# TomClabault/RayTracerCPP

Hardware: AMD Instinct MI355X
Metric: Mrays/sec (primary+shadow) at 1920x1080, 1M-tri scene; max |dpixel| (higher is better)
Workload: dtype f32; 1 GPU; C4 sphere1m: 1,000,000 tris, 1920x1080, ssaa_factor 2 (3840x2160 rays), primary + shadow, octree 12/40; rays_per_frame=10029157, primary_rays=8294400, reflection_rays=0, band_rows=8, parallelism=image strips x1, frames_in_flight=3, world_size=1, bands=interleaved b % N

## Files before the change

### __graft_entry__.py

```python
import os
import subprocess
import sys

ROOT = os.path.dirname(os.path.abspath(__file__))


def _make(args, cwd):
    jobs = str(min(8, os.cpu_count() or 1))
    subprocess.run(["make", "-j" + jobs] + args, cwd=cwd, check=True)


def build() -> None:
    _make([], os.path.join(ROOT, "raytracercpp_amd", "csrc"))
    _make([], os.path.join(ROOT, "oracle"))
    if os.path.isdir("/root/reference/tp2"):
        _make(["ref", "ref_v3"], os.path.join(ROOT, "oracle"))
    sys.path.insert(0, ROOT)
    import raytracercpp_amd
    from raytracercpp_amd import _lib
    _lib.lib()
    sys.path.insert(0, os.path.join(ROOT, "tests"))
    from test_c_api import build_c_program
    build_c_program()
    from scene_bound_tool import build_program
    build_program()
    from tile_mask_tool import build_program as build_tile_mask_program
    build_tile_mask_program()
    if os.path.isdir("/root/reference/tp2"):
        from test_reference_adapter import build_adapter_program
        build_adapter_program()


def smoke() -> None:
    sys.path.insert(0, ROOT)
    import numpy as np
    from raytracercpp_amd import scenes
    from raytracercpp_amd.renderer import Renderer
    from oracle.bindings import Oracle

    sc, st = scenes.bumpy70k(width=160, height=90)
    r = Renderer(0)
    r.load_scene(sc, st)
    r.request_aux(hit=True)
    ref = Oracle(sc, st).render_rows()
    for frame in ("octree", "wide BVH"):
        r.ray_trace()
        r.post_process()
        img = r.get_image().ravel()
        gpu = r.get_internal(argb=False, hit=True)
        assert np.array_equal(gpu["hit_id"], ref.hit_id), f"hit-ID mismatch vs oracle ({frame} frame)"
        assert np.array_equal(img, ref.argb), f"ARGB mismatch vs oracle ({frame} frame)"
        r.finish_accel()
    print("smoke OK:", r.stats())
```

### include/rt_mi355x.h

```cpp
#ifndef RT_MI355X_H
#define RT_MI355X_H

#include <stdint.h>

#ifdef __cplusplus
extern "C" {
#endif

#define RT_OK 0
#define RT_EINVAL (-1)
#define RT_EHIP (-2)
#define RT_ENOMEM (-3)
#define RT_ESTATE (-4)
#define RT_EUNSUPPORTED (-5)
#define RT_EIO (-6)

#define RT_SHADING_RT 0
#define RT_SHADING_ABS_NORMALS 1
#define RT_SHADING_PASTEL_NORMALS 2
#define RT_SHADING_BARYCENTRIC 3
#define RT_SHADING_VISUALIZE_AO 4

#define RT_TEX_AO 0
#define RT_TEX_DIFFUSE 1
// ... 114 lines not shown
int rt_get_camera_matrices(rt_renderer *r, float pos[3], float proj_inv[16], float cam_to_world[16]);

int rt_set_camera_projection(rt_renderer *r, const float proj[16], const float world_to_cam[16]);

int rt_set_camera_lens(rt_renderer *r, float fov, float aspect);

int rt_set_object_transform(rt_renderer *r, const float m[16]);
int rt_reset_previous_transform(rt_renderer *r);
int rt_get_triangles(rt_renderer *r, float *tri9, int64_t *n);

int rt_set_texture(rt_renderer *r, int32_t slot, int32_t w, int32_t h, const float *rgba);

int rt_set_skybox(rt_renderer *r, const int32_t w[6], const int32_t h[6], const float *const faces[6]);

int rt_reconstruct_bvh_new(rt_renderer *r);
int rt_destroy_bvh(rt_renderer *r);

int rt_ray_trace(rt_renderer *r);

int rt_raster_trace(rt_renderer *r);

int rt_get_ssao_buffers(rt_renderer *r, float *z, float *n4, int32_t *ao);

int rt_post_process(rt_renderer *r);

int rt_get_image(rt_renderer *r, uint32_t *argb, int32_t *w, int32_t *h);

int rt_lock_image(rt_renderer *r);
int rt_unlock_image(rt_renderer *r);

int rt_render(rt_renderer *r, float *ms);

int rt_request_aux(rt_renderer *r, int32_t want_rgba, int32_t want_hit, int32_t want_shadow);
int rt_get_internal(rt_renderer *r, uint32_t *argb, float *rgba, int32_t *hit_id, float *hit_t, uint8_t *shadow);

int rt_get_stats(rt_renderer *r, rt_stats *out);

int rt_local_rows(rt_renderer *r, int32_t band_rows, int32_t rank, int32_t nranks, int32_t *rows_out);
int rt_render_bands_device(rt_renderer *r, int32_t band_rows, int32_t rank, int32_t nranks, uint32_t *d_out,
                           void *hip_stream);
int rt_render_band_list_device(rt_renderer *r, int32_t band_rows, const int32_t *bands, int32_t nbands,
                               uint32_t *d_out, void *hip_stream);
int rt_band_costs(rt_renderer *r, void *hip_stream, double *costs, int32_t nbands);

int rt_trace_rays(rt_renderer *r, const float *orig, const float *dir, int64_t n, int32_t *tri_id, float *t,
                  float *u, float *v, uint8_t *ret);

int rt_trace_ray(rt_renderer *r, const float *orig, const float *dir, int64_t n, int32_t current_recursion_depth,
                 float *rgba, int32_t *hit_src, float *t, uint8_t *intersection_found, uint8_t *shadowed);

int rt_kernel_times(rt_renderer *r, float *ms, int32_t n);
int rt_band_counters(rt_renderer *r, int64_t *shadow_rays, int64_t *reflection_rays);
int rt_tile_mask(rt_renderer *r, int32_t src, uint32_t *words, int64_t cap, int32_t info[5]);

void rt_make_transform(int32_t kind, float x, float y, float z, float out[16]);
void rt_compose(const float a[16], const float b[16], float out[16]);
void rt_inverse(const float m[16], float out[16]);
void rt_perspective(float fov, float aspect, float znear, float zfar, float out[16]);
void rt_transform_points(const float m[16], const float *pts, int64_t n, float *out);

typedef struct rt_obj rt_obj;
rt_obj *rt_obj_open(const char *path, const float xform[16], int32_t mat_offset);
int rt_obj_counts(const rt_obj *o, int64_t *ntri, int32_t *nmat, int32_t *has_uv);
int rt_obj_fetch(const rt_obj *o, float *tri9, int32_t *mat, float *uv6, float *mats16);
void rt_obj_close(rt_obj *o);


#ifdef __cplusplus
}
#endif
#endif
```

### include/rt_mi355x_diag.h

```cpp
#ifndef RT_MI355X_DIAG_H
#define RT_MI355X_DIAG_H

#include "rt_mi355x.h"

#ifdef __cplusplus
extern "C" {
#endif

int rt_debug_read(rt_renderer *r, uint64_t *out, int64_t n);
int rt_tile_costs(rt_renderer *r, uint32_t *out, int64_t n, int32_t *tiles_x, int32_t *tiles_y);

int rt_wide_query(rt_renderer *r, const float *orig, const float *dir, int64_t n, int32_t kind, float *o_out,
                  float *d_out, int32_t *status, int32_t *tri_id, float *t, float *u, float *v, uint8_t *shadowed);
int rt_risk_words(rt_renderer *r, int32_t src, uint64_t *out, int64_t cap, int64_t *count, int64_t *violations);

int rt_octree_digest(const float *tri9, int64_t n, int32_t max_depth, int32_t leaf_max_obj_count, int32_t builder,
                     uint64_t *digest, int64_t stats[7], float *ms);

int rt_wbvh_query(const float *tri9, int64_t n, int32_t max_depth, int32_t leaf_max_obj_count, const float *orig,
                  const float *dir, int64_t nrays, int32_t *status, int32_t *id, float *t, float *u, float *v,
                  int64_t stats[8], float *ms);
int rt_wbvh_query_ex(const float *tri9, int64_t n, int32_t max_depth, int32_t leaf_max_obj_count, const float *orig,
                     const float *dir, int64_t nrays, const float *cam, const float *light, int32_t shadow_rays,
                     float *o_out, float *d_out, int32_t *status, int32_t *id, float *t, float *u, float *v,
                     int64_t stats[8], float *ms, int32_t *ray_nodes, int32_t ocone_dim, int64_t oc_stats[5]);

int rt_ocone_check(const float *tri9, int64_t n, int32_t max_depth, int32_t leaf_max_obj_count, int32_t ocone_dim,
                   const float *orig, const float *dir, int64_t nrays, int32_t *skip, int64_t out[6],
                   const uint32_t *cells, const int32_t *dims, const float *lo_ih, uint32_t *cells_out);
int rt_ocone_read(rt_renderer *r, uint32_t *out, int64_t n, int32_t dims[3], float lo_ih[4]);
int rt_risk_cap_check(const float *tri9, int64_t n, int32_t max_depth, int32_t leaf_max_obj_count, const float *cam,
                      const float *dir, int64_t nrays, float cap_override, int32_t *skip, int64_t out[4]);

#ifdef __cplusplus
}
#endif
#endif
```

### raytracercpp_amd/_lib.py

```python
from __future__ import annotations

import ctypes as C
import os

import numpy as np

HERE = os.path.dirname(os.path.abspath(__file__))
LIB_PATH = os.path.join(HERE, "librt_mi355x.so")
if os.environ.get("RT_LIB_PATH"):
    LIB_PATH = os.environ["RT_LIB_PATH"]

RT_OK = 0
ERRORS = {-1: "RT_EINVAL", -2: "RT_EHIP", -3: "RT_ENOMEM", -4: "RT_ESTATE", -5: "RT_EUNSUPPORTED", -6: "RT_EIO"}

_f32p = C.POINTER(C.c_float)
_i32p = C.POINTER(C.c_int32)
_u32p = C.POINTER(C.c_uint32)
_u8p = C.POINTER(C.c_uint8)
_i64p = C.POINTER(C.c_int64)


class RtSettings(C.Structure):
    _fields_ = [
        ("image_width", C.c_int32), ("image_height", C.c_int32),
        ("enable_ssaa", C.c_int32), ("ssaa_factor", C.c_int32),
        ("enable_clipping", C.c_int32), ("hybrid_rasterization_tracing", C.c_int32),
        ("shading_method", C.c_int32), ("compute_shadows", C.c_int32), ("max_recursion_depth", C.c_int32),
        ("enable_bvh", C.c_int32), ("bvh_max_depth", C.c_int32), ("bvh_leaf_object_count", C.c_int32),
        ("enable_ssao", C.c_int32), ("ssao_sample_count", C.c_int32),
        ("ssao_radius", C.c_float), ("ssao_amount", C.c_float),
        ("enable_ambient", C.c_int32), ("enable_diffuse", C.c_int32), ("enable_specular", C.c_int32),
        ("enable_emissive", C.c_int32), ("rough_reflections_sample_count", C.c_int32),
        ("enable_ao_mapping", C.c_int32), ("enable_diffuse_mapping", C.c_int32),
        ("enable_normal_mapping", C.c_int32), ("enable_displacement_mapping", C.c_int32),
        ("displacement_mapping_strength", C.c_float), ("parallax_mapping_steps", C.c_int32),
        ("enable_roughness_mapping", C.c_int32), ("enable_skysphere", C.c_int32), ("enable_skybox", C.c_int32),
        ("rng_seed", C.c_uint32),
    ]


class RtStats(C.Structure):
    _fields_ = [
        ("primary_rays", C.c_int64), ("shadow_rays", C.c_int64), ("reflection_rays", C.c_int64),
        ("kernel_ms", C.c_float), ("post_ms", C.c_float), ("build_ms", C.c_float),
        ("octree_inner", C.c_int64), ("octree_leaves", C.c_int64), ("octree_empty_leaves", C.c_int64),
        ("octree_max_leaf", C.c_int64), ("octree_max_depth", C.c_int64),
        ("gpu_nodes", C.c_int64), ("gpu_tris", C.c_int64),
        ("render_width", C.c_int32), ("render_height", C.c_int32), ("seg_scale", C.c_float),
        ("work", C.c_int64 * 4), ("work_wide", C.c_int64 * 4), ("uncertified", C.c_int64 * 6),
        ("wave_steps", C.c_int64 * 6), ("build_split_ms", C.c_float * 4), ("host_builds", C.c_int64),
        ("wide_tree", C.c_int32),
    ]

    def as_dict(self):
        def conv(n, t):
            v = getattr(self, n)
            if t is C.c_float:
                return float(v)
            if isinstance(v, C.Array):
                return [float(x) if n == "build_split_ms" else int(x) for x in v]
            return int(v)
        return {n: conv(n, t) for n, t in self._fields_}


_H = C.c_void_p
SIGNATURES = {
    "rt_default_settings": (None, [C.POINTER(RtSettings)]),
    "rt_create": (_H, [C.c_int]),
    "rt_destroy": (None, [_H]),
    "rt_last_error": (C.c_char_p, []),
    "rt_get_settings": (C.c_int, [_H, C.POINTER(RtSettings)]),
    "rt_set_settings": (C.c_int, [_H, C.POINTER(RtSettings)]),
    "rt_change_render_size": (C.c_int, [_H, C.c_int32, C.c_int32]),
    "rt_set_exact": (C.c_int, [_H, C.c_int]),
    "rt_finish_accel": (C.c_int, [_H]),
    "rt_set_devices": (C.c_int, [_H, _i32p, C.c_int32]),
    "rt_set_triangles": (C.c_int, [_H, _f32p, _i32p, _f32p, C.c_int64]),
    "rt_add_sphere": (C.c_int, [_H, C.c_float, C.c_float, C.c_float, C.c_float, C.c_int32]),
    "rt_add_plane": (C.c_int, [_H] + [C.c_float] * 6 + [C.c_int32]),
    "rt_clear_geometry": (C.c_int, [_H]),
    "rt_set_materials": (C.c_int, [_H, _f32p, C.c_int32]),
    "rt_get_material_count": (C.c_int, [_H, _i32p]),
    "rt_change_camera_fov": (C.c_int, [_H, C.c_float]),
    "rt_change_camera_aspect_ratio": (C.c_int, [_H, C.c_float]),
    "rt_set_light_position": (C.c_int, [_H, C.c_float, C.c_float, C.c_float]),
    "rt_set_camera_transform": (C.c_int, [_H, _f32p]),
    "rt_apply_transformation_to_camera": (C.c_int, [_H, _f32p]),
    "rt_set_camera_matrices": (C.c_int, [_H, _f32p, _f32p, _f32p]),
    "rt_set_camera_projection": (C.c_int, [_H, _f32p, _f32p]),
    "rt_set_camera_lens": (C.c_int, [_H, C.c_float, C.c_float]),
    "rt_get_ssao_buffers": (C.c_int, [_H, _f32p, _f32p, _i32p]),
    "rt_get_camera_matrices": (C.c_int, [_H, _f32p, _f32p, _f32p]),
    "rt_set_object_transform": (C.c_int, [_H, _f32p]),
    "rt_reset_previous_transform": (C.c_int, [_H]),
    "rt_get_triangles": (C.c_int, [_H, _f32p, _i64p]),
    "rt_get_device_transforms": (C.c_int, [_H, _i64p]),
    "rt_transform_points_device": (C.c_int, [C.c_int32, _f32p, _f32p, C.c_int64, _f32p, _i32p, _f32p]),
    "rt_set_triangles_device": (C.c_int, [_H, C.c_void_p, C.c_int64, C.c_void_p, _i32p, _f32p, C.c_int64, C.c_void_p]),
    "rt_update_vertices_device": (C.c_int, [_H, C.c_void_p, C.c_int64, C.c_void_p, C.c_void_p]),
    "rt_get_device_ingests": (C.c_int, [_H, _i64p]),
    "rt_gather_triangles_device": (C.c_int, [C.c_int32, _f32p, C.c_int64, _i32p, C.c_int64, _f32p, _i32p, _f32p]),
    "rt_set_accel_deferred": (C.c_int, [_H, C.c_int]),
    "rt_get_accel_builds": (C.c_int, [_H, _i64p]),
    "rt_set_texture": (C.c_int, [_H, C.c_int32, C.c_int32, C.c_int32, _f32p]),
    "rt_set_skybox": (C.c_int, [_H, _i32p, _i32p, C.POINTER(_f32p)]),
    "rt_reconstruct_bvh_new": (C.c_int, [_H]),
    "rt_destroy_bvh": (C.c_int, [_H]),
    "rt_ray_trace": (C.c_int, [_H]),
    "rt_raster_trace": (C.c_int, [_H]),
    "rt_post_process": (C.c_int, [_H]),
    "rt_get_image": (C.c_int, [_H, _u32p, _i32p, _i32p]),
    "rt_render": (C.c_int, [_H, _f32p]),
    "rt_lock_image": (C.c_int, [_H]),
    "rt_unlock_image": (C.c_int, [_H]),
    "rt_request_aux": (C.c_int, [_H, C.c_int32, C.c_int32, C.c_int32]),
    "rt_get_internal": (C.c_int, [_H, _u32p, _f32p, _i32p, _f32p, _u8p]),
    "rt_get_stats": (C.c_int, [_H, C.POINTER(RtStats)]),
    "rt_local_rows": (C.c_int, [_H, C.c_int32, C.c_int32, C.c_int32, _i32p]),
    "rt_render_bands_device": (C.c_int, [_H, C.c_int32, C.c_int32, C.c_int32, C.c_void_p, C.c_void_p]),
    "rt_render_band_list_device": (C.c_int, [_H, C.c_int32, _i32p, C.c_int32, C.c_void_p, C.c_void_p]),
    "rt_band_costs": (C.c_int, [_H, C.c_void_p, C.POINTER(C.c_double), C.c_int32]),
    "rt_trace_rays": (C.c_int, [_H, _f32p, _f32p, C.c_int64, _i32p, _f32p, _f32p, _f32p, _u8p]),
    "rt_trace_ray": (C.c_int, [_H, _f32p, _f32p, C.c_int64, C.c_int32, _f32p, _i32p, _f32p, _u8p, _u8p]),
    "rt_wide_query": (C.c_int, [_H, _f32p, _f32p, C.c_int64, C.c_int32, _f32p, _f32p, _i32p, _i32p, _f32p, _f32p, _f32p,
                                _u8p]),
    "rt_risk_words": (C.c_int, [_H, C.c_int32, C.POINTER(C.c_uint64), C.c_int64, _i64p, _i64p]),
    "rt_kernel_times": (C.c_int, [_H, _f32p, C.c_int32]),
    "rt_band_counters": (C.c_int, [_H, _i64p, _i64p]),
    "rt_tile_mask": (C.c_int, [_H, C.c_int32, _u32p, C.c_int64, _i32p]),
    "rt_make_transform": (None, [C.c_int32, C.c_float, C.c_float, C.c_float, _f32p]),
    "rt_compose": (None, [_f32p, _f32p, _f32p]),
    "rt_inverse": (None, [_f32p, _f32p]),
    "rt_perspective": (None, [C.c_float, C.c_float, C.c_float, C.c_float, _f32p]),
    "rt_transform_points": (None, [_f32p, _f32p, C.c_int64, _f32p]),
    "rt_obj_open": (_H, [C.c_char_p, _f32p, C.c_int32]),
    "rt_obj_counts": (C.c_int, [_H, _i64p, _i32p, _i32p]),
    "rt_obj_fetch": (C.c_int, [_H, _f32p, _i32p, _f32p, _f32p]),
    "rt_obj_close": (None, [_H]),
    "rt_octree_digest": (C.c_int, [_f32p, C.c_int64, C.c_int32, C.c_int32, C.c_int32, C.POINTER(C.c_uint64), _i64p,
                                   _f32p]),
    "rt_octree_build_device": (C.c_int, [C.c_int32, _f32p, C.c_int64, C.c_int32, C.c_int32, C.POINTER(C.c_uint64),
                                         _i64p, _f32p]),
    "rt_set_device_build": (C.c_int, [_H, C.c_int]),
    "rt_get_device_builds": (C.c_int, [_H, _i64p]),
    "rt_get_device_wide_builds": (C.c_int, [_H, _i64p]),
    "rt_wbvh_quick_digest": (C.c_int, [_f32p, C.c_int64, C.c_int32, C.c_int32, C.POINTER(C.c_uint64), _i64p, _f32p]),
    "rt_wbvh_quick_build_device": (C.c_int, [C.c_int32, _f32p, C.c_int64, C.c_int32, C.c_int32, C.POINTER(C.c_uint64),
                                             _i64p, _i64p, _f32p]),
    "rt_debug_read": (C.c_int, [_H, C.POINTER(C.c_uint64), C.c_int64]),
    "rt_tile_costs": (C.c_int, [_H, C.POINTER(C.c_uint32), C.c_int64, _i32p, _i32p]),
    "rt_wbvh_query": (C.c_int, [_f32p, C.c_int64, C.c_int32, C.c_int32, _f32p, _f32p, C.c_int64, _i32p, _i32p, _f32p,
                                _f32p, _f32p, _i64p, _f32p]),
    "rt_wbvh_query_ex": (C.c_int, [_f32p, C.c_int64, C.c_int32, C.c_int32, _f32p, _f32p, C.c_int64, _f32p, _f32p,
                                   C.c_int32, _f32p, _f32p, _i32p, _i32p, _f32p, _f32p, _f32p, _i64p, _f32p, _i32p,
                                   C.c_int32, _i64p]),
    "rt_ocone_check": (C.c_int, [_f32p, C.c_int64, C.c_int32, C.c_int32, C.c_int32, _f32p, _f32p, C.c_int64, _i32p,
                                 _i64p, C.POINTER(C.c_uint32), _i32p, _f32p, C.POINTER(C.c_uint32)]),
    "rt_ocone_read": (C.c_int, [_H, C.POINTER(C.c_uint32), C.c_int64, _i32p, _f32p]),
    "rt_risk_cap_check": (C.c_int, [_f32p, C.c_int64, C.c_int32, C.c_int32, _f32p, _f32p, C.c_int64, C.c_float, _i32p,
                                    _i64p]),
}

GEOMETRY_INPUT = ("rt_set_triangles_device", "rt_update_vertices_device", "rt_get_device_ingests",
                  "rt_gather_triangles_device", "rt_set_accel_deferred", "rt_get_accel_builds")

_lib = None


def has(name):
    return hasattr(lib(), name)


def lib():
    global _lib
    if _lib is None:
        if not os.path.exists(LIB_PATH):
            raise RuntimeError(f"{LIB_PATH} is missing: the HIP library must be built "
                               "(python -c 'import __graft_entry__ as g; g.build()')")
        try:
            import torch
        except ImportError:
            pass
        L = C.CDLL(LIB_PATH)
        for name, (res, args) in SIGNATURES.items():
            if name in GEOMETRY_INPUT and os.environ.get("RT_LIB_PATH") and not hasattr(L, name):
                continue
            fn = getattr(L, name)
            fn.restype = res
            fn.argtypes = args
        _lib = L
    return _lib


class RtError(RuntimeError):
    def __init__(self, code, where):
        msg = lib().rt_last_error()
        super().__init__(f"{where}: {ERRORS.get(code, code)}: {msg.decode() if msg else ''}")
        self.code = code


def check(rc, where):
    if rc != RT_OK:
        raise RtError(rc, where)
    return rc


def ptr(a, t):
    if a is None:
# ... 76 lines not shown


def device_geometry_args(verts, indices, device):
    import torch

    def form(t, name, dtype, cols):
        if not isinstance(t, torch.Tensor):
            raise TypeError(f"{name}: a torch tensor on the GPU is needed, not {type(t).__name__}")
        if t.dtype != dtype:
            raise TypeError(f"{name}: dtype {t.dtype}, {dtype} is needed")
        if t.dim() != 2 or t.shape[1] != cols:
            raise ValueError(f"{name}: shape {tuple(t.shape)}, [n, {cols}] is needed")

    def place(t, name):
        if not t.is_cuda:
            raise ValueError(f"{name}: the tensor is on {t.device}, not on a GPU")
        if t.device.index != int(device):
            raise ValueError(f"{name}: the tensor is on GPU {t.device.index}, the renderer on GPU {int(device)}")
        if not t.is_contiguous():
            raise ValueError(f"{name}: the tensor is not contiguous")

    form(verts, "verts", torch.float32, 9 if indices is None else 3)
    if indices is not None:
        form(indices, "indices", torch.int32, 3)
    place(verts, "verts")
    if indices is None:
        return verts.data_ptr(), 3 * verts.shape[0], None, verts.shape[0]
    place(indices, "indices")
    return verts.data_ptr(), verts.shape[0], indices.data_ptr(), indices.shape[0]


def load_obj(path, xform, mat_offset=0):
    xform = f32(xform)
    L = lib()
    h = L.rt_obj_open(path.encode(), ptr(xform, _f32p), mat_offset)
    if not h:
        raise RuntimeError(f"rt_obj_open({path}): {L.rt_last_error().decode()}")
    try:
        n = C.c_int64()
        nm = C.c_int32()
        has_uv = C.c_int32()
        check(L.rt_obj_counts(h, C.byref(n), C.byref(nm), C.byref(has_uv)), "rt_obj_counts")
        tri = np.zeros((n.value, 9), np.float32)
        mat = np.zeros(n.value, np.int32)
        uv = np.zeros((n.value, 6), np.float32) if has_uv.value else None
        mats = np.zeros((nm.value, 16), np.float32)
        check(L.rt_obj_fetch(h, ptr(tri, _f32p), ptr(mat, _i32p), ptr(uv, _f32p), ptr(mats, _f32p)), "rt_obj_fetch")
        return tri, mat, uv, mats
    finally:
        L.rt_obj_close(h)


def wbvh_query(tri9, orig, dirs, max_depth=12, leaf=40, cam=None, light=None, shadow_rays=False, rays_out=False,
               ray_nodes=None, ocone_dim=0, oc_stats=None):
    tri9 = f32(tri9).reshape(-1, 9)
    o = f32(orig).reshape(-1, 3)
    d = f32(dirs).reshape(-1, 3)
    n = o.shape[0]
    st = np.zeros(n, np.int32)
    ids = np.zeros(n, np.int32)
    t, u, v = (np.zeros(n, np.float32) for _ in range(3))
    stats = np.zeros(8, np.int64)
    ms = np.zeros(2, np.float32)
    oo = np.zeros((n, 3), np.float32)
    do = np.zeros((n, 3), np.float32)
    c = None if cam is None else f32(cam).reshape(3)
    li = None if light is None else f32(light).reshape(3)
    check(lib().rt_wbvh_query_ex(ptr(tri9, _f32p), tri9.shape[0], max_depth, leaf, ptr(o, _f32p), ptr(d, _f32p), n,
                                 None if c is None else ptr(c, _f32p), None if li is None else ptr(li, _f32p),
                                 1 if shadow_rays else 0, ptr(oo, _f32p), ptr(do, _f32p),
                                 ptr(st, _i32p), ptr(ids, _i32p), ptr(t, _f32p), ptr(u, _f32p), ptr(v, _f32p),
                                 ptr(stats, _i64p), ptr(ms, _f32p),
                                 None if ray_nodes is None else ptr(ray_nodes, _i32p), int(ocone_dim),
                                 None if oc_stats is None else ptr(oc_stats, _i64p)), "rt_wbvh_query")
    keys = ("nodes", "leaves", "max_leaf", "depth", "node_visits", "tri_tests", "violations", "sah_x1000")
    out = (st, ids, t, u, v, dict(zip(keys, map(int, stats))), (float(ms[0]), float(ms[1])))
    return out + (oo, do) if rays_out else out


def ocone_check(tri9, orig, dirs, max_depth=12, leaf=40, ocone_dim=64, grid=None, want_cells=False):
    tri9 = f32(tri9).reshape(-1, 9)
    o = f32(orig).reshape(-1, 3)
    d = f32(dirs).reshape(-1, 3)
    skip = np.zeros(o.shape[0], np.int32)
    out = np.zeros(6, np.int64)
    _u32p = C.POINTER(C.c_uint32)
    cells = dims = lo_ih = None
    if grid is not None:
        cells = np.ascontiguousarray(grid[0], np.uint32)
        dims = np.ascontiguousarray(grid[1], np.int32)
        lo_ih = f32(grid[2])
    built = None
    if want_cells:
        built = np.zeros(((ocone_dim + 2) ** 3, 2), np.uint32)
    check(lib().rt_ocone_check(ptr(tri9, _f32p), tri9.shape[0], max_depth, leaf, ocone_dim, ptr(o, _f32p),
                               ptr(d, _f32p), o.shape[0], ptr(skip, _i32p), ptr(out, _i64p),
                               None if cells is None else ptr(cells, _u32p), None if dims is None else ptr(dims, _i32p),
                               None if lo_ih is None else ptr(lo_ih, _f32p), None if built is None else ptr(built, _u32p)),
          "rt_ocone_check")
    keys = ("violations", "skipping", "grazing_tests", "cells", "empty_cells", "noskip_cells")
    res = (skip, dict(zip(keys, map(int, out))))
    return res + (built,) if want_cells else res


def risk_cap_check(tri9, cam, dirs, max_depth=12, leaf=40, cap_override=-1.0):
    tri9 = f32(tri9).reshape(-1, 9)
    c = f32(cam).reshape(3)
    d = f32(dirs).reshape(-1, 3)
    skip = np.zeros(d.shape[0], np.int32)
    out = np.zeros(4, np.int64)
    check(lib().rt_risk_cap_check(ptr(tri9, _f32p), tri9.shape[0], max_depth, leaf, ptr(c, _f32p), ptr(d, _f32p),
                                  d.shape[0], float(cap_override), ptr(skip, _i32p), ptr(out, _i64p)), "rt_risk_cap_check")
    return skip, {"violations": int(out[0]), "skipping": int(out[1]), "grazing_tests": int(out[2]),
                  "cap": float(out[3]) * 1e-9 if out[3] >= 0 else None}


def octree_digest(tri9, max_depth=12, leaf=40, builder=0):
    tri9 = f32(tri9).reshape(-1, 9)
    dg = C.c_uint64()
    st = np.zeros(7, np.int64)
    ms = C.c_float()
    check(lib().rt_octree_digest(ptr(tri9, _f32p), tri9.shape[0], max_depth, leaf, builder, C.byref(dg),
                                 ptr(st, _i64p), C.byref(ms)), "rt_octree_digest")
    keys = ("inner", "leaves", "empty_leaves", "max_leaf", "max_depth", "nodes", "levels")
    return int(dg.value), dict(zip(keys, map(int, st))), float(ms.value)


# ... 37 lines not shown
```

### raytracercpp_amd/csrc/capi.cpp

```cpp
#include <atomic>
#include <chrono>
#include <cmath>
#include <thread>
#include <cstring>
#include <new>
#include <string>

#include "../../include/rt_mi355x_diag.h"
#include "host_scene.hpp"
#include "launch.hpp"
#include "octree.hpp"
#include "octree_gpu.hpp"
#include "ocone.hpp"
#include "wbvh.hpp"
#include "wbvh_quick_gpu.hpp"
#include "renderer.hpp"

namespace {
thread_local std::string g_err;

int record(rt::Renderer* r, int rc)
{
    if (rc != RT_OK)
        g_err = r->error();
// ... 396 lines not shown
        *rows_out = n;
        return RT_OK;
    });
}
int rt_render_bands_device(rt_renderer* r, int32_t band_rows, int32_t rank, int32_t nranks, uint32_t* d_out,
                           void* hip_stream)
{
    return guarded(R(r), [&] {
        return R(r)->render_bands_device(band_rows, rank, nranks, d_out, reinterpret_cast<hipStream_t>(hip_stream));
    });
}

int rt_render_band_list_device(rt_renderer* r, int32_t band_rows, const int32_t* bands, int32_t nbands, uint32_t* d_out,
                               void* hip_stream)
{
    return guarded(R(r), [&] {
        return R(r)->render_band_list_device(band_rows, bands, nbands, d_out, reinterpret_cast<hipStream_t>(hip_stream));
    });
}
int rt_band_costs(rt_renderer* r, void* hip_stream, double* costs, int32_t nbands)
{
    return guarded(R(r), [&] { return R(r)->band_costs(reinterpret_cast<hipStream_t>(hip_stream), costs, nbands); });
}

int rt_trace_rays(rt_renderer* r, const float* orig, const float* dir, int64_t n, int32_t* tri_id, float* t,
                  float* u, float* v, uint8_t* ret)
{
    return guarded(R(r), [&] { return R(r)->trace_rays(orig, dir, n, tri_id, t, u, v, ret); });
}
int rt_wide_query(rt_renderer* r, const float* orig, const float* dir, int64_t n, int32_t kind, float* o_out,
                  float* d_out, int32_t* status, int32_t* tri_id, float* t, float* u, float* v, uint8_t* shadowed)
{
    return guarded(R(r), [&] { return R(r)->wide_query(orig, dir, n, kind, o_out, d_out, status, tri_id, t, u, v, shadowed); });
}
int rt_risk_words(rt_renderer* r, int32_t src, uint64_t* out, int64_t cap, int64_t* count, int64_t* violations)
{
    return guarded(R(r), [&] { return R(r)->risk_words(src, out, cap, count, violations); });
}
int rt_trace_ray(rt_renderer* r, const float* orig, const float* dir, int64_t n, int32_t current_recursion_depth,
                 float* rgba, int32_t* hit_src, float* t, uint8_t* intersection_found, uint8_t* shadowed)
{
    return guarded(R(r), [&] {
        return R(r)->trace_ray_colors(orig, dir, n, current_recursion_depth, rgba, hit_src, t, intersection_found,
                                      shadowed);
    });
}
int rt_kernel_times(rt_renderer* r, float* ms, int32_t n)
{
    return guarded(R(r), [&] { return ms ? R(r)->kernel_times(ms, n) : RT_EINVAL; });
}
int rt_tile_mask(rt_renderer* r, int32_t src, uint32_t* words, int64_t cap, int32_t info[5])
{
    return guarded(R(r), [&] { return info ? R(r)->tile_mask(src, words, cap, info) : RT_EINVAL; });
}
int rt_band_counters(rt_renderer* r, int64_t* shadow_rays, int64_t* reflection_rays)
{
    return guarded(R(r), [&] {
        unsigned long long c[2] = {0, 0};
        int rc = R(r)->band_counters(c);
        if (shadow_rays) *shadow_rays = (int64_t)c[0];
        if (reflection_rays) *reflection_rays = (int64_t)c[1];
        return rc;
    });
}

void rt_make_transform(int32_t kind, float x, float y, float z, float out[16])
{
    switch (kind) {
    case 0: rt::mat::translation(x, y, z, out); break;
    case 1: rt::mat::rotation_x(x, out); break;
    case 2: rt::mat::rotation_y(x, out); break;
    case 3: rt::mat::rotation_z(x, out); break;
    case 4: rt::mat::scale(x, y, z, out); break;
    default: rt::mat::identity(out); break;
    }
}
void rt_compose(const float a[16], const float b[16], float out[16]) { rt::mat::compose(a, b, out); }
void rt_inverse(const float m[16], float out[16]) { rt::mat::inverse(m, out); }
void rt_perspective(float fov, float aspect, float znear, float zfar, float out[16])
{
    rt::mat::perspective(fov, aspect, znear, zfar, out);
}
void rt_transform_points(const float m[16], const float* pts, int64_t n, float* out)
{
    rt::mat::transform_points(m, pts, n, out);
}

struct rt_obj {
    rt::ObjData data;
};

rt_obj* rt_obj_open(const char* path, const float xform[16], int32_t mat_offset)
{
    try {
        float ident[16];
        rt::mat::identity(ident);
        rt_obj* o = new rt_obj;
        std::string err;
        if (!rt::load_obj(path, xform ? xform : ident, mat_offset, o->data, err)) {
            g_err = err;
            delete o;
            return nullptr;
        }
        return o;
    } catch (const std::exception& e) {
        g_err = e.what();
// ... 618 lines not shown
            return hip_bad(e, "readback");
        if (info.tris &&
            ((e = hipMemcpy(f.tris.data(), d_tris.p, f.tris.size() * sizeof(rt::GTri), hipMemcpyDeviceToHost)) != hipSuccess ||
             (e = hipMemcpy(f.tri_id.data(), d_tri_id.p, f.tri_id.size() * 4, hipMemcpyDeviceToHost)) != hipSuccess))
            return hip_bad(e, "readback");
        rt::WBvh w;
        const size_t np = (size_t)st[0], nt = (size_t)st[2];
        w.nodes.resize(np);
        w.slot.resize(nt);
        w.leaf_of_slot.resize(nt);
        w.tri_leaf.resize(nt);
        w.parent.resize(np);
        if (np && ((e = hipMemcpy(w.nodes.data(), d_wnodes.p, np * sizeof(rt::WNode), hipMemcpyDeviceToHost)) != hipSuccess ||
                   (e = hipMemcpy(w.slot.data(), d_wtmp.p, nt * 4, hipMemcpyDeviceToHost)) != hipSuccess ||
                   (e = hipMemcpy(w.leaf_of_slot.data(), d_wtmp.as<char>() + nt * 4, nt * 4, hipMemcpyDeviceToHost)) != hipSuccess ||
                   (e = hipMemcpy(w.tri_leaf.data(), d_wlinks.p, nt * 4, hipMemcpyDeviceToHost)) != hipSuccess ||
                   (e = hipMemcpy(w.parent.data(), d_wlinks.as<char>() + nt * 4, np * 4, hipMemcpyDeviceToHost)) != hipSuccess))
            return hip_bad(e, "readback");
        w.leaf_of_k.resize(nt);
        for (size_t k = 0; k < nt; k++)
            w.leaf_of_k[k] = (size_t)w.slot[k] < nt ? w.leaf_of_slot[(size_t)w.slot[k]] : 0u;
        w.stats.nodes = st[0];
        w.stats.leaves = st[1];
        w.stats.tris = st[2];
        w.stats.max_leaf = st[3];
        w.stats.depth = st[4];
        wquick_report(w, digest, stats);
        rt::WBvh host;
        rt::build_wbvh_quick(f, host, true);
        wquick_compare(w, host, check);
        bool slots_ok = true;
        for (size_t k = 0; k < nt; k++) slots_ok = slots_ok && w.slot[k] >= 0 && (size_t)w.slot[k] < nt;
        if (np && slots_ok) {
            rt::wbvh_fill_tris(f, w);
            check[0] = rt::check_wbvh(f, w);
        } else
            check[0] = np ? 1 : 0;
        if (ms) {
            ms[0] = dev_ms;
            ms[1] = std::chrono::duration<float, std::milli>(std::chrono::steady_clock::now() - t0).count();
        }
        return RT_OK;
    } catch (const std::bad_alloc&) {
        g_err = "rt_wbvh_quick_build_device: out of host memory";
        return RT_ENOMEM;
    }
}

int rt_wbvh_query(const float* tri9, int64_t n, int32_t max_depth, int32_t leaf_max_obj_count, const float* orig,
                  const float* dir, int64_t nrays, int32_t* status, int32_t* id, float* t, float* u, float* v,
                  int64_t stats[8], float* ms)
{
    return rt_wbvh_query_ex(tri9, n, max_depth, leaf_max_obj_count, orig, dir, nrays, nullptr, nullptr, 0, nullptr,
                            nullptr, status, id, t, u, v, stats, ms, nullptr, 0, nullptr);
}

int rt_wbvh_query_ex(const float* tri9, int64_t n, int32_t max_depth, int32_t leaf_max_obj_count, const float* orig,
                     const float* dir, int64_t nrays, const float* cam, const float* light, int32_t shadow_rays,
                     float* o_out, float* d_out, int32_t* status, int32_t* id, float* t, float* u, float* v,
                     int64_t stats[8], float* ms, int32_t* ray_nodes, int32_t ocone_dim, int64_t oc_stats[5])
{
    if (n < 0 || (n > 0 && !tri9) || nrays < 0 || (nrays > 0 && (!orig || !dir || !status || !id || !t || !u || !v)) ||
        (shadow_rays && !light))
        return bad("rt_wbvh_query: bad arguments");
    try {
        rt::FlatOctree f;
        rt::WBvh w;
        auto t0 = std::chrono::steady_clock::now();
        rt::build_flat_octree(tri9, n, max_depth, leaf_max_obj_count, f);
        auto t1 = std::chrono::steady_clock::now();
        rt::build_wbvh(f, w);
        if (ms) {
            ms[0] = std::chrono::duration<float, std::milli>(t1 - t0).count();
            ms[1] = std::chrono::duration<float, std::milli>(std::chrono::steady_clock::now() - t1).count();
        }
        float S = 0.0f;
        if (!f.nodes.empty())
            for (int a = 0; a < 3; a++)
                S = std::max(S, std::max(std::fabs(f.nodes[0].dn[a]), std::fabs(f.nodes[0].df[a])));
        const bool usable = !w.nodes.empty() && S > 0x1p-20f && S < 0x1p20f;
        std::vector<uint64_t> risk;
        rt::WRiskArgs RA{};
        float cap[2] = {-1.0f, -1.0f};
        float cap_dir[2][3] = {};
        if (usable && (cam || light)) {
            const float lo[3] = {f.nodes[0].dn[0], f.nodes[0].dn[1], f.nodes[0].dn[2]};
            const float hi[3] = {f.nodes[0].df[0], f.nodes[0].df[1], f.nodes[0].df[2]};
            const float zero[3] = {0, 0, 0};
            RA = rt::wbvh_risk_args(lo, hi, S, cam ? cam : zero, light ? light : zero, W_QS_CLOSEST, W_QS_SHADOW);
            risk.assign(w.nodes.size() * 8, rt::wrisk_pack(INFINITY, 0));
            std::vector<float> lbox(6 * w.tris.size());
            for (size_t k = 0; k < w.tris.size(); k++) {
                const rt::GNode& L = f.nodes[w.leaf_of_k[k]];
                for (int a = 0; a < 3; a++) {
                    lbox[6 * k + a] = L.dn[a];
                    lbox[6 * k + 3 + a] = L.df[a];
                }
            }
            if (cam)
                rt::wbvh_risk_host(w, lbox, RA, 0, risk);
            if (light)
                rt::wbvh_risk_host(w, lbox, RA, 1, risk);
            if (std::getenv("RT_RISK_CAP") == nullptr || std::atoi(std::getenv("RT_RISK_CAP")) != 0)
                for (int sel = 0; sel < 2; sel++) {
                    if (!RA.on[sel] || (sel == 0 ? !cam : !light))
                        continue;
                    const float* X = sel == 0 ? cam : light;
                    double v[3], l = 0;
                    for (int a = 0; a < 3; a++) {
                        v[a] = 0.5 * ((double)lo[a] + (double)hi[a]) - (double)X[a];
                        l += v[a] * v[a];
                    }
                    l = std::sqrt(l);
                    for (int a = 0; a < 3; a++)
                        cap_dir[sel][a] = l > 0 && l < INFINITY ? (float)(v[a] / l) : (a == 0 ? 1.0f : 0.0f);
                    const double c[3] = {cap_dir[sel][0], cap_dir[sel][1], cap_dir[sel][2]};
                    float sm = INFINITY;
                    for (const rt::GTri& t : w.tris)
                        if (rt::wbvh_risk_key(t, RA.p[sel][0], RA.p[sel][1], RA.p[sel][2], RA.G[sel], RA.nu[sel],
                                              RA.slack[sel], RA.QS[sel]) < INFINITY)
                            sm = std::min(sm, rt::risk_cap_tri(t, c));
                    cap[sel] = sm;
                }
        }
        rt::OConeGrid ocg;
        rt::OConeView ocv{};
        if (usable && ocone_dim > 0) {
            rt::build_origin_cones(w, S, W_QS_CLOSEST, 0.0102 + 0x1p-16 * S, ocone_dim, 80.0 * 3.14159265358979 / 180.0, 0, ocg);
            if (!ocg.cells.empty()) {
                ocv.cells = ocg.cells.data();
                for (int a = 0; a < 3; a++) {
                    ocv.lo[a] = ocg.lo[a];
                    ocv.dim[a] = ocg.dim[a];
                }
                ocv.ih = ocg.ih;
            }
        }
        std::atomic<int64_t> work_n{0}, work_t{0}, n_nob{0};
        const bool probe_hi = std::getenv("RT_WQ_PROBE_HI") != nullptr;
        auto body = [&](int64_t b, int64_t e) {
            rt::WStackLocal stk;
            uint32_t wk[4] = {0, 0, 0, 0};
            for (int64_t i = b; i < e; i++) {
                rt::v3 o = rt::mk(orig[3 * i], orig[3 * i + 1], orig[3 * i + 2]);
                rt::v3 d = rt::mk(dir[3 * i], dir[3 * i + 1], dir[3 * i + 2]);
                const uint64_t* rk = nullptr;
                int rsel = 0;
                float rsub = 0.0f;
                if (shadow_rays) {
                    const rt::v3 p = o, nrm = d, lp = rt::mk(light[0], light[1], light[2]);
                    o = p + nrm * 1.0e-4f;
                    d = rt::normalize(lp - p);
                    const float nl = std::fabs(nrm.x) + std::fabs(nrm.y) + std::fabs(nrm.z);
                    const float hi = (std::sqrt(rt::length2(p - lp)) + 1.0e-4f * nl) * (1.0f + 0x1p-10f);
                    if (!risk.empty() && hi <= RA.ray_G && nl <= RA.ray_nl) {
                        rk = risk.data();
                        rsel = 1;
                        rsub = rt::wrisk_sub(W_QS_SHADOW, hi, RA.ray_nu);
                    }
                } else if (!risk.empty() && cam && o.x == cam[0] && o.y == cam[1] && o.z == cam[2])
                    rk = risk.data();
                if (o_out) {
                    o_out[3 * i] = o.x;
                    o_out[3 * i + 1] = o.y;
                    o_out[3 * i + 2] = o.z;
                }
                if (d_out) {
                    d_out[3 * i] = d.x;
                    d_out[3 * i + 1] = d.y;
                    d_out[3 * i + 2] = d.z;
                }
                bool nan = false;
                for (int p = 0; p < rt::NPLANES; p++) {
                    rt::v3 pn = rt::mk(rt::PLANE_N[p][0], rt::PLANE_N[p][1], rt::PLANE_N[p][2]);
                    float den = rt::dot(pn, d), num = rt::dot(pn, o);
                    nan |= den != den || num != num;
                }
                id[i] = -1;
                t[i] = -1.0f;
                u[i] = 1.0f;
                v[i] = 0.0f;
                if (f.nodes.empty()) {
                    status[i] = rt::W_MISS;
                    continue;
                }
                if (!usable || nan) {
                    status[i] = rt::W_UNCERT;
                    continue;
                }
                float om = std::max(std::fabs(o.x), std::max(std::fabs(o.y), std::fabs(o.z)));
                float m = 0x1p-16f * (om + S);
                rt::WHit h;
                const uint32_t wk0 = wk[0];
                bool nob = !shadow_rays && !rk && rt::ocone_skip(ocv, o, d, W_QS_CLOSEST);
                if (rk && !shadow_rays && cap[0] >= 0.0f)
                    nob = rt::risk_cap_skip(cap[0], cap_dir[0], d, W_QS_CLOSEST);
                if (rk && shadow_rays && cap[1] >= 0.0f)
                    nob = rt::risk_cap_skip(cap[1], cap_dir[1], d, W_QS_SHADOW);
                if (nob)
                    ++n_nob;
                int st = rt::wbvh_closest(w.nodes.data(), w.tris.data(), o, d, m, stk, h, wk, INFINITY, true,
                                          shadow_rays ? W_QS_SHADOW : W_QS_CLOSEST, rk, rsel, rsub, 0u,
                                          (rt::WNoFeed*)nullptr, nob);
                if (st == rt::W_DEEP) {
                    rt::WStackArr<rt::W_DEEP_STACK> deep;
                    st = rt::wbvh_closest(w.nodes.data(), w.tris.data(), o, d, m, deep, h, wk, INFINITY, true,
                                          shadow_rays ? W_QS_SHADOW : W_QS_CLOSEST, rk, rsel, rsub);
                    if (st == rt::W_DEEP)
                        st = rt::W_UNCERT;
                }
                if (st == rt::W_HIT && probe_hi) {
                    rt::WStackArr<rt::W_DEEP_STACK> deep;
                    rt::WHit h2;
                    wk[0] = wk0;
                    rt::wbvh_closest(w.nodes.data(), w.tris.data(), o, d, m, deep, h2, wk, h.t, true,
                                     shadow_rays ? W_QS_SHADOW : W_QS_CLOSEST, rk, rsel, rsub);
                }
                if (st == rt::W_HIT) {
                    int32_t slot = w.slot[(size_t)h.k];
                    if (rt::kdop_certifies(f.nodes[w.leaf_of_slot[(size_t)slot]], o, d, h.t)) {
                        id[i] = f.tri_id[(size_t)slot];
                        t[i] = h.t;
                        u[i] = h.u;
                        v[i] = h.v;
                    } else
                        st = rt::W_UNCERT;
                }
                status[i] = st;
                if (ray_nodes)
                    ray_nodes[i] = (int32_t)(wk[0] - wk0);
            }
            work_n += wk[0];
            work_t += wk[1];
        };
        unsigned hc = std::max(1u, std::min(std::thread::hardware_concurrency(), 16u));
        std::vector<std::thread> th;
        int64_t chunk = (nrays + hc - 1) / hc;
        for (unsigned k = 0; k < hc; k++) {
            int64_t b = (int64_t)k * chunk, e = std::min(nrays, b + chunk);
            if (b < e)
                th.emplace_back(body, b, e);
        }
        for (auto& x : th)
            x.join();
        if (stats) {
            stats[0] = w.stats.nodes;
            stats[1] = w.stats.leaves;
            stats[2] = w.stats.max_leaf;
            stats[3] = w.stats.depth;
            stats[4] = work_n.load();
            stats[5] = work_t.load();
            stats[6] = rt::check_wbvh(f, w);
            if (!risk.empty()) {
                if (cam)
                    stats[6] += rt::check_risk_words(f, w, RA, 0, risk.data());
                if (light)
// ... 20 lines not shown
```

### raytracercpp_amd/csrc/kernels.hip

```cpp
#include <hip/hip_runtime.h>
#include <stdint.h>
#if defined(RT_COUNT) && RT_COUNT
__device__ unsigned long long g_wsteps[8];
__device__ __forceinline__ void w_step_hook(uint32_t cur, int leaf)
{
    const uint64_t act = __ballot(1);
    uint64_t left = act;
    unsigned distinct = 0;
    while (left) {
        const uint32_t f = (uint32_t)__builtin_amdgcn_readlane((int)cur, __ffsll((unsigned long long)left) - 1);
        left &= ~__ballot(cur == f);
        distinct++;
    }
    if ((int)__lane_id() == __ffsll((unsigned long long)act) - 1) {
        atomicAdd(&g_wsteps[2 * leaf], 1ull);
        if (distinct == 1)
            atomicAdd(&g_wsteps[2 * leaf + 1], 1ull);
        atomicAdd(&g_wsteps[4 + leaf], (unsigned long long)__popcll(act));
        atomicAdd(&g_wsteps[6 + leaf], (unsigned long long)distinct);
    }
}
#define W_STEP_HOOK(cur, leaf) w_step_hook(cur, leaf)
#endif
#include "kparams.hpp"
// ... 738 lines not shown
template <int N = W_STACK>
struct WStackLdsN {
    static constexpr int CAP = N;
    uint2* base;
    __device__ __forceinline__ void put(int i, uint2 v) { base[i * BLOCK] = v; }
    __device__ __forceinline__ uint2 get(int i) const { return base[i * BLOCK]; }
    __device__ __forceinline__ uint2 get_lane(int delta, int i) const { return base[delta + i * BLOCK]; }
};
using WStackLds = WStackLdsN<W_STACK>;

#if RT_COUNT
__device__ void count_wave_steps(const KParams& P, int base, uint32_t steps)
{
    if (!P.counters)
        return;
    uint64_t act = __ballot(1), a = act;
    uint32_t mx = 0;
    while (a) {
        const int l = __ffsll((unsigned long long)a) - 1;
        a &= a - 1;
        mx = max(mx, (uint32_t)__builtin_amdgcn_readlane((int)steps, l));
    }
    if ((int)__lane_id() == __ffsll((unsigned long long)act) - 1) {
        atomicAdd(&P.counters[base], (unsigned long long)mx);
        atomicAdd(&P.counters[base + 2], 1ull);
    }
    atomicAdd(&P.counters[base + 1], (unsigned long long)steps);
}
#endif


struct WDeep {
    int st;
    WHit w;
};
__device__ __noinline__ WDeep wide_closest_deep(const WNode* wnodes, const GTri* wtris, v3 o, v3 d, float m, float hi,
                                                bool ties, float QS, const uint64_t* rk, int rsel, float rsub)
{
    WStackArr<W_DEEP_STACK> stk;
    WDeep r;
    const int st = wbvh_closest(wnodes, wtris, o, d, m, stk, r.w, nullptr, hi, ties, QS, rk, rsel, rsub);
    r.st = st == W_DEEP ? W_UNCERT : st;
    return r;
}

__device__ __forceinline__ float wide_margin(const KParams& P, v3 o)
{
    const float om = fmaxf(fabsf(o.x), fmaxf(fabsf(o.y), fabsf(o.z)));
    return 0x1p-16f * (om + P.scene_scale);
}

template <class Stk, int G>
__device__ __forceinline__ int wide_run(const KParams& P, v3 o, v3 d, uint2* lv, WHit& w, float hi, bool ties, float QS,
                                        const uint64_t* rk, int rsel, float rsub, uint32_t max_steps, bool nob, int count)
{
    const float m = wide_margin(P, o);
    Stk stk{lv};
#if RT_COUNT
    uint32_t work[4] = {0, 0, 0, 0};
    uint32_t* wk = count >= 0 ? work : nullptr;
#else
    uint32_t* wk = nullptr;
#endif
    int st = wbvh_closest<Stk, G>(P.wnodes, P.wtris, o, d, m, stk, w, wk, hi, ties, QS, rk, rsel, rsub, max_steps,
                                  (WNoFeed*)nullptr, nob);
#if RT_COUNT
    if (wk) {
        count_wave_steps(P, count, wk[3]);
        if (P.counters) {
            atomicAdd(&P.counters[10], (unsigned long long)wk[0]);
            atomicAdd(&P.counters[11], (unsigned long long)wk[1]);
            for (int c = 0; c < 5; c++)
                if ((wk[2] >> c) & 1u)
                    atomicAdd(&P.counters[16 + c], 1ull);
        }
    }
#endif
    if (st == W_DEEP) {
        const WDeep r = wide_closest_deep(P.wnodes, P.wtris, o, d, m, hi, ties, QS, rk, rsel, rsub);
        st = r.st;
        w = r.w;
    }
    return st;
}

__device__ __forceinline__ bool wide_certified(const KParams& P, const WHit& w, v3 o, v3 d, uint4& M)
{
    M = ldg(P.wmeta + w.k);
    return kdop_certifies(load_gnode(P.nodes + M.y), o, d, w.t);
}

template <int G = 1, int CAP = W_STACK>
__device__ __forceinline__ bool wide_closest(const KParams& P, v3 o, v3 d, THit& h, bool& r, uint2* lv,
                                             Rec* rec = nullptr, uint32_t max_steps = 0, bool* longq = nullptr)
{
    using Stk = WStackLdsN<G == 1 ? CAP : W_STACK>;
    WHit w;
    const bool cam = o.x == P.cam_pos[0] && o.y == P.cam_pos[1] && o.z == P.cam_pos[2];
    const uint64_t* rk = P.wrisk && cam ? P.wrisk : nullptr;
    const bool nob = rk && P.risk_cap && risk_cap_skip(P.risk_cap[0], P.cap_dir[0], d, W_QS_CLOSEST);
    int st = W_MISS;
    if (!(cam && P.sb_valid && scene_bound_rejects(P.sb_lo, P.sb_hi, o, d)))
        st = wide_run<Stk, G>(P, o, d, lv, w, INFINITY, true, W_QS_CLOSEST, rk, 0, 0.0f, RT_COUNT ? 0u : max_steps, nob, 22);
    if (max_steps && st == W_LONG) {
        *longq = true;
        return false;
    }
    if (st == W_MISS) {
        h.t = -1.0f;
        h.u = 1.0f;
        h.v = 0.0f;
        h.k = -1;
        r = false;
        return true;
    }
#if RT_COUNT
    if (st == W_HIT && P.counters)
        atomicAdd(&P.counters[14], 1ull);
#endif
    uint4 M;
    if (st == W_HIT && wide_certified(P, w, o, d, M)) {
        h.t = w.t;
        h.u = w.u;
        h.v = w.v;
        h.k = (int32_t)M.x;
        r = true;
        if (rec)
            *rec = rec_of(P, load_gtri(P.wtris + w.k), (int)M.z, (int)M.w, h);
        return true;
    }
#if RT_COUNT
    if (P.counters) {
        atomicAdd(&P.counters[12], 1ull);
        if (st == W_HIT)
            atomicAdd(&P.counters[21], 1ull);
    }
#endif
    return false;
}

template <int G = 1, int CAP = W_STACK>
__device__ __forceinline__ bool wide_shadow(const KParams& P, v3 o, v3 d, float hi, v3 p, v3 lp, uint2* lv, bool* sh,
                                            bool light)
{
    using Stk = WStackLdsN<G == 1 ? CAP : W_STACK>;
    WHit w;
    const uint64_t* rk = light ? P.wrisk : nullptr;
    const float rsub = light ? wrisk_sub(W_QS_SHADOW, hi, P.risk_nu) : 0.0f;
    static_assert(W_QS_SHADOW <= W_QS_CLOSEST, "the origin cones hold the at-risk triangles for the larger split");
    const bool nob = ocone_skip(P.ocone, o, d, W_QS_SHADOW) || (light && P.risk_cap && risk_cap_skip(P.risk_cap[1], P.cap_dir[1], d, W_QS_SHADOW));
    const int st = wide_run<Stk, G>(P, o, d, lv, w, hi, false, W_QS_SHADOW, rk, 1, rsub, 0u, nob, 25);
    if (st == W_MISS) {
        *sh = false;
        return true;
    }
#if RT_COUNT
// ... 117 lines not shown
        const OctQ oq = octree_query<CALL>(P, o, d, 0.0f, 0.0f, false, lv);
        h = oq.h;
        r = oq.r;
        if (r) {
            v3 q = o + d * h.t;
            if (length2(p - q) < length2(p - lp))
                return true;
        }
    } else {
        TRay R = make_ray(P, o, d);
        h.t = -1.0f;
        for (int k = 0; k < P.ntri_slots; k++) {
            float t, u, v;
            if (tri_test(P.tris, (uint32_t)k, R, t, u, v)) {
                h.t = t;
                v3 q = o + d * h.t;
                if (length2(p - q) < length2(p - lp))
                    return true;
            }
        }
    }
    if (PLAIN)
        return false;
    return shapes_shadow(P, o, d, h.t, p, lp);
}

__device__ __forceinline__ c3 background() { return col(135.0f / 255.0f, 206.0f / 255.0f, 235.0f / 255.0f); }

__device__ __forceinline__ void bvh_record(const KParams& P, const THit& h, bool r, Rec& local, Rec& fin, int& src)
{
    if (h.k >= 0)
        local = tri_record(P, h);
    else
        local.t = h.t != h.t ? h.t : local.t;
    if (r && (local.t < fin.t || fin.t == -1)) {
        fin = local;
        src = local.tri;
    }
}

__device__ __forceinline__ void shapes_closest(const KParams& P, v3 o, v3 d, Rec& local, Rec& fin, int& src)
{
    for (int k = 0; k < P.nshape; k++) {
        bool hk = P.shape_kind[k] == 0 ? sphere_test(P.shape[k], P.shape_mat[k], o, d, local)
                                       : plane_test(P.shape[k], P.shape_mat[k], o, d, local);
        if (hk && (local.t < fin.t || fin.t == -1)) {
            fin = local;
            src = -2 - k;
        }
    }
}

template <bool PLAIN = false, int G = 1, bool OCT = false>
__device__ int closest_hit(const KParams& P, v3 o, v3 d, Rec& fin, uint2* lv)
{
    Rec local = rec_fresh();
    int src = -1;
    if (PLAIN || P.enable_bvh) {
        THit h;
        bool r = false;
        const bool wide = !OCT && P.wnodes && P.nnodes > 0 && !ray_is_nan(o, d);
        if (wide && wide_closest<G, PLAIN ? W_STACK_PLAIN : W_STACK>(P, o, d, h, r, lv, &local)) {
            if (r && (local.t < fin.t || fin.t == -1)) {
                fin = local;
                src = local.tri;
            }
        } else {
            const OctQ q = octree_query<PLAIN && !OCT>(P, o, d, 0.0f, 0.0f, false, lv);
            bvh_record(P, q.h, q.r, local, fin, src);
        }
    } else {
        TRay R = make_ray(P, o, d);
        THit best, last;
        best.k = -1;
        last.k = -1;
        float bt = fin.t;
        for (int k = 0; k < P.ntri_slots; k++) {
            float t, u, v;
            if (tri_test(P.tris, (uint32_t)k, R, t, u, v)) {
                last.t = t; last.u = u; last.v = v; last.k = k;
                if (t < bt || bt == -1) {
                    bt = t;
                    best = last;
                }
            }
        }
        if (best.k >= 0) {
            fin = tri_record(P, best);
            src = fin.tri;
        }
        if (last.k >= 0)
            local = tri_record(P, last);
    }
    if (!PLAIN)
        shapes_closest(P, o, d, local, fin, src);
    return src;
}

struct Direct {
    c3 fc;
    v3 ip;
    bool shadowed;
};

template <bool PLAIN = false>
__device__ c3 shade_lit(const KParams& P, v3 ro, v3 rd, Rec& h, v3& ip_out)
{
    c3 fc = col(0.0f, 0.0f, 0.0f);
    float u = h.u, v = h.v;
    v3 ip = ro + rd * h.t;
    ip_out = ip;
    v3 cam = mk(P.cam_pos[0], P.cam_pos[1], P.cam_pos[2]);
    v3 light = mk(P.light[0], P.light[1], P.light[2]);
    if (!PLAIN && P.enable_displacement_mapping)
        parallax_occlusion_mapping(P, h.tri, h.u, h.v, normalize(cam - ip), u, v);
// ... 119 lines not shown
}

__device__ __forceinline__ uint32_t mix32(uint32_t x)
{
    x ^= x >> 16; x *= 0x7feb352dU;
    x ^= x >> 15; x *= 0x846ca68bU;
    x ^= x >> 16;
    return x;
}

__device__ __forceinline__ uint32_t sample_state(uint32_t key, uint32_t i)
{
    uint32_t x = mix32(key ^ (0x9E3779B9u * (2u * i + 1u)));
    return x ? x : 0x9E3779B9u;
}

__device__ __forceinline__ uint32_t child_key(uint32_t key, uint32_t i)
{
    return mix32(key ^ (0x85EBCA6Bu * (2u * i + 2u)));
}

__device__ __forceinline__ float rng_bilateral(uint32_t& s)
{
    uint32_t x = s;
    x ^= x << 13;
    x ^= x >> 17;
    x ^= x << 5;
    s = x;
    return (float)x / (float)UINT32_MAX * 2 - 1;
}

struct Frame {
    c3 fc;
    c3 total;
    v3 ro, perfect, n;
    float rough;
    int mat, i, sc;
    uint32_t key;
    Rec rhi;
};

constexpr int MAX_FRAMES = 16;

struct PixelOut {
    c3 color;
    float alpha;
    Rec fin;
    int src;
    bool found, shadowed;
};

template <bool REFL, bool PLAIN = false, int G = 1, bool OCT = false>
__device__ PixelOut trace_pixel(const KParams& P, v3 cam, v3 rd0, uint2* lv, uint32_t pixel_key, unsigned& nshadow,
                                unsigned& nrefl)
{
    PixelOut po;
    po.fin = rec_fresh();
    po.found = po.shadowed = false;
    po.alpha = 1.0f;
    po.src = closest_hit<PLAIN && !REFL, REFL ? 1 : G, OCT>(P, cam, rd0, po.fin, lv);
    if (PLAIN) PH_MARK(2);
    if (!REFL) {
        if (PLAIN && po.fin.t > 0.1f) {
            po.found = true;
            v3 ip;
            const c3 fc = shade_lit<true>(P, cam, rd0, po.fin, ip);
            if (P.compute_shadows)
                nshadow++;
            uint2* sv = lv + (size_t)lds_save_slot_plain<OCT>(P) * BLOCK;
            sv[0] = make_uint2(fbits(fc.r), fbits(fc.g));
            sv[BLOCK] = make_uint2(fbits(fc.b), (uint32_t)po.fin.mat);
            sv[2 * BLOCK] = make_uint2(fbits(po.fin.t), (uint32_t)po.src);
            asm volatile("" ::: "memory");
            const v3 light = mk(P.light[0], P.light[1], P.light[2]);
            if (PLAIN) PH_MARK(3);
            po.shadowed = is_shadowed<true, G, !OCT, OCT>(P, ip, po.fin.normal, light, lv);
            if (PLAIN) PH_MARK(4);
            asm volatile("" ::: "memory");
            const uint2 s0 = sv[0], s1 = sv[BLOCK], s2 = sv[2 * BLOCK];
            po.fin.mat = (int)s1.y;
            po.fin.t = bitsf(s2.x);
            po.src = (int)s2.y;
            const float* m = mat_of(P, po.fin.mat);
            po.color = shade_finish(P, shade_shadow_emit(P, col(bitsf(s0.x), bitsf(s0.y), bitsf(s1.x)), m, po.shadowed), m,
                                    col(0, 0, 0));
            return po;
        }
        if (po.fin.t > 0.1f) {
            po.found = true;
            Direct D = shade_direct<PLAIN, G, OCT>(P, cam, rd0, po.fin, lv, nshadow);
            po.shadowed = D.shadowed;
            po.color = PLAIN || P.shading_method == RT_SHADING
                           ? shade_finish(P, D.fc, mat_of(P, po.fin.mat), col(0, 0, 0))
                           : clamp3(D.fc);
        } else
            po.color = miss_color<PLAIN>(P, rd0, po.alpha);
        return po;
    }

    Frame fr[MAX_FRAMES];
    const int N = P.rough_reflections_sample_count;
    enum { S_TRACE, S_RET, S_NEXT };
    int state, depth = 0, f = 0;
    v3 ro = cam, rd = rd0;
    c3 ret = col(0, 0, 0);
    bool first = true;
    uint32_t next_key = pixel_key;
    state = S_TRACE;
    for (;;) {
        if (state == S_TRACE) {
            Rec& fin = depth == 0 ? po.fin : fr[depth - 1].rhi;
            if (depth > P.max_recursion_depth) {
                ret = col(0.0f, 0.0f, 0.0f);
// ... 273 lines not shown
    case 1: __builtin_amdgcn_s_setprio(1); break;
    default: __builtin_amdgcn_s_setprio(0); break;
    }
}

template <int G = 1, int C0 = 8>
__device__ __forceinline__ void downscale_tile(const KParams& P, int lane, int lr, int px, uint32_t c, int C = C0)
{
    int r = (int)((c >> 16) & 0xffu), g = (int)((c >> 8) & 0xffu), b = (int)(c & 0xffu);
    const int f = 1 << P.ds_shift;
    for (int m = 1; m < f; m <<= 1) {
        r += __shfl_xor(r, G * m);
        g += __shfl_xor(g, G * m);
        b += __shfl_xor(b, G * m);
    }
    for (int m = C; m < C * f; m <<= 1) {
        r += __shfl_xor(r, G * m);
        g += __shfl_xor(g, G * m);
        b += __shfl_xor(b, G * m);
    }
    const int pl = lane / G;
    if ((lane & (G - 1)) == 0 && ((pl % C) & (f - 1)) == 0 && ((pl / C) & (f - 1)) == 0) {
        const int s2 = 2 * P.ds_shift;
        P.ds_out[(size_t)(lr >> P.ds_shift) * (size_t)(P.rw >> P.ds_shift) + (size_t)(px >> P.ds_shift)] =
            qrgb(r >> s2, g >> s2, b >> s2);
    }
}

__device__ __forceinline__ v3 camera_dir(const KParams& P, int px, int py, v3 cam)
{
    const float y_world = ((float)py + 0.5f) / P.rh * 2 - 1;
    const float x_world = ((float)px + 0.5f) / P.rw * 2 - 1;
    v3 vs;
    if (P.proj_mode != 0) {
        const float* m = P.proj_inv;
        const float x = x_world, y = y_world, z = -1.0f;
        const float xt = m[0] * x + m[1] * y + m[2] * z + m[3];
        const float yt = m[4] * x + m[5] * y + m[6] * z + m[7];
        const float zt = m[8] * x + m[9] * y + m[10] * z + m[11];
        const float w = P.proj_w;
        vs = P.proj_mode == 1 ? mk(xt, yt, zt) : mk(xt * w, yt * w, zt * w);
    } else
        vs = xform_point(P.proj_inv, mk(x_world, y_world, -1));
    v3 ws;
    if (P.c2w_affine && fabsf(vs.x) < INFINITY && fabsf(vs.y) < INFINITY && fabsf(vs.z) < INFINITY) {
        const float* m = P.cam_to_world;
        ws = mk(m[0] * vs.x + m[1] * vs.y + m[2] * vs.z + m[3], m[4] * vs.x + m[5] * vs.y + m[6] * vs.z + m[7],
                m[8] * vs.x + m[9] * vs.y + m[10] * vs.z + m[11]);
    } else
        ws = xform_point(P.cam_to_world, vs);
    return normalize(ws - cam);
}

template <int G>
__device__ __forceinline__ void trace_split_part(const KParams& P, uint2* lv, int t, int lane, unsigned& nshadow)
{
    static_assert(G > 1 && G <= 8 && (G & (G - 1)) == 0, "2, 4 or 8 lanes per pixel");
    const int cap = P.tiles_x * P.tiles_y / 16;
    const int np = P.split_parts;
    const int tq = ldg(P.heavy_list + cap + t / np), part = t % np;
    const int tile = tq & 0x0fffffff;
    set_wave_prio(tq >> 28);
    const uint64_t t0 = __builtin_amdgcn_s_memtime();
    int tx, ty;
    tile_xy(P, tile, tx, ty);
    const int npix = 64 / np;
    const int C = npix >= 16 ? 8 : npix / 2, R = npix / C;
    const int pl = lane / G;
    const int px = tx * 8 + (part % (8 / C)) * C + pl % C;
    const int lr = ty * 8 + (part / (8 / C)) * R + pl / C;
    const int py = lr < P.local_rows ? global_row(P, lr) : P.rh;
    if (pl < npix && px < P.rw && py < P.rh) {
        const v3 cam = mk(P.cam_pos[0], P.cam_pos[1], P.cam_pos[2]);
        const v3 rd = camera_dir(P, px, py, cam);
        unsigned ns = 0, nr = 0;
        PixelOut po = trace_pixel<false, true, G>(P, cam, rd, lv, 0u, ns, nr);
        if ((lane & (G - 1)) == 0)
            nshadow += ns;
        const size_t o = (size_t)lr * P.rw + px;
        const uint32_t c = color_to_argb(po.color);
        if (P.ds_out) downscale_tile<G>(P, lane, lr, px, c, C);
        if ((lane & (G - 1)) == 0) {
            if (P.argb) P.argb[o] = c;
            if (P.rgba) P.rgba[o] = make_float4(po.color.r, po.color.g, po.color.b, po.alpha);
            if (P.hit_id) P.hit_id[o] = po.found ? po.src : -1;
            if (P.hit_t) P.hit_t[o] = po.fin.t;
            if (P.shadow) P.shadow[o] = (uint8_t)(po.found && po.shadowed);
        }
    }
    const uint64_t c = __builtin_amdgcn_s_memtime() - t0;
    if (lane == 0) {
        const uint32_t c32 = c > 0xFFFFFFFFull ? 0xFFFFFFFFu : (uint32_t)c;
        atomicAdd(P.tile_cost + tile, c32);
        tile_stats_add(c32, c32 > 0xFFFFFFFFu / G ? 0xFFFFFFFFu : c32 * G);
    }
}

__device__ __forceinline__ void tile_cost_store(const KParams& P, int tile, uint64_t t0, int lane)
{
    const uint64_t c = __builtin_amdgcn_s_memtime() - t0;
    if (lane == 0) {
        const uint32_t c32 = c > 0xFFFFFFFFull ? 0xFFFFFFFFu : (uint32_t)c;
        P.tile_cost[tile] = c32;
        tile_stats_add(c32, c32);
    }
}

__device__ __noinline__ void fill_masked_tile(const KParams& P, int lr, int px)
{
    const c3 bg = background();
    const uint32_t c = color_to_argb(bg);
    const size_t o = (size_t)lr * P.rw + px;
    if (P.argb) P.argb[o] = c;
    if (P.ds_out) {
        const int f = 1 << P.ds_shift;
        if ((px & (f - 1)) == 0 && (lr & (f - 1)) == 0)
            P.ds_out[(size_t)(lr >> P.ds_shift) * (size_t)(P.rw >> P.ds_shift) + (size_t)(px >> P.ds_shift)] =
                qrgb((int)((c >> 16) & 0xffu), (int)((c >> 8) & 0xffu), (int)(c & 0xffu));
    }
    if (P.rgba) P.rgba[o] = make_float4(bg.r, bg.g, bg.b, 1.0f);
    if (P.hit_id) P.hit_id[o] = -1;
    if (P.hit_t) P.hit_t[o] = rec_fresh().t;
    if (P.shadow) P.shadow[o] = (uint8_t)0;
#if RT_COUNT
    if (P.counters && (threadIdx.x & 63) == 0)
        atomicAdd(&P.counters[28], 1ull);
#endif
}

// ... 14 lines not shown
        g_phase[threadIdx.x >> 6][7] = __builtin_amdgcn_s_memtime();
    }
#endif
    for (;;) {
        auto kpl = kp;
        asm volatile("" : "+s"(kpl));
        const KParams& P = *reinterpret_cast<const KParams*>((const void*)kpl);
        const v3 cam = mk(P.cam_pos[0], P.cam_pos[1], P.cam_pos[2]);
        if (PLAIN && !REFL && !OCT && P.heavy_group == SPLIT_G &&
            !__builtin_amdgcn_readfirstlane(__hip_atomic_load(&g_bq.split_done, __ATOMIC_RELAXED, __HIP_MEMORY_SCOPE_WORKGROUP))) {
            int t = 0;
            if (lane == 0)
                t = atomicAdd(P.heavy_ctr + 2, 1);
            t = __builtin_amdgcn_readfirstlane(t);
            if (t < P.split_parts * min(ldg(P.heavy_ctr + 3), P.tiles_x * P.tiles_y / 16)) {
                trace_split_part<SPLIT_G>(P, lv, t, lane, nshadow);
                continue;
            }
            if (lane == 0)
                __hip_atomic_store(&g_bq.split_done, 1, __ATOMIC_RELAXED, __HIP_MEMORY_SCOPE_WORKGROUP);
        }
        const int tq = tile_queue_next(P);
        if (PLAIN) PH_MARK(6);
        if (tq < 0)
            break;
        const int tile = tq & 0x0fffffff;
        if (P.heavy_list)
            set_wave_prio(tq >> 28);
        const uint64_t tile_t0 = __builtin_amdgcn_s_memtime();
        int tx, ty;
        tile_xy(P, tile, tx, ty);
        int px = tx * 8 + (lane & 7);
        int lr = ty * 8 + (lane >> 3);
        int py = lr < P.local_rows ? global_row(P, lr) : P.rh;
        if (PLAIN) PH_MARK(0);
        if (px >= P.rw || py >= P.rh) {
            if (P.tile_cost && lane == 0)
                P.tile_cost[tile] = 0u;
            continue;
        }
        if (PLAIN && !REFL && !OCT && P.tile_mask) {
            const uint32_t mw = ldg(P.tile_mask + (size_t)(py >> 3) * (size_t)P.mask_wpr + (size_t)(px >> 8));
            if (!__ballot((mw >> ((px >> 3) & 31)) & 1u)) {
                fill_masked_tile(P, lr, px);
                if (P.tile_cost)
                    tile_cost_store(P, tile, tile_t0, lane);
                continue;
            }
        }
        const v3 rd = camera_dir(P, px, py, cam);
        if (PLAIN) PH_MARK(1);

        uint32_t rng = REFL ? pixel_seed((uint32_t)(py * P.rw + px), P.rng_seed) : 0u;
        PixelOut po = trace_pixel<REFL, PLAIN, 1, OCT>(P, cam, rd, lv, rng, nshadow, nrefl);
        size_t o = (size_t)lr * P.rw + px;
        if (P.argb) P.argb[o] = color_to_argb(po.color);
        if (!REFL && P.ds_out) downscale_tile(P, lane, lr, px, color_to_argb(po.color));
        if (P.rgba) P.rgba[o] = make_float4(po.color.r, po.color.g, po.color.b, po.alpha);
        if (P.hit_id) P.hit_id[o] = po.found ? po.src : -1;
        if (P.hit_t) P.hit_t[o] = po.fin.t;
        if (P.shadow) P.shadow[o] = (uint8_t)(po.found && po.shadowed);
        if (!PLAIN && P.zbuf) write_ssao_buffers(P, o, po.found, cam, rd, po.fin);
        if (PLAIN) PH_MARK(5);
        if (P.tile_cost)
            tile_cost_store(P, tile, tile_t0, lane);
    }
    tile_stats_flush(P, lane);
#if RT_PHASE_TIME
    if (PLAIN) {
        PH_MARK(0);
        const int wid = (int)(blockIdx.x * WAVES_PER_BLOCK + (threadIdx.x >> 6));
        if (P.dbg && lane == 0 && wid < DBG_WAVES)
            for (int k = 0; k < 7; k++)
                P.dbg[DBG_WORDS * wid + k] = g_phase[threadIdx.x >> 6][k];
    }
#endif
    if (nshadow) atomicAdd(&P.counters[0], (unsigned long long)nshadow);
    if (nrefl) atomicAdd(&P.counters[1], (unsigned long long)nrefl);
}

__device__ __forceinline__ v3 ld3(const float* p) { return mk(p[0], p[1], p[2]); }
__device__ __forceinline__ void st3(float* p, v3 v) { p[0] = v.x; p[1] = v.y; p[2] = v.z; }
__device__ __forceinline__ void st3(float* p, c3 c) { p[0] = c.r; p[1] = c.g; p[2] = c.b; }
__device__ __forceinline__ c3 ldc(const float* p) { return col(p[0], p[1], p[2]); }

__device__ __forceinline__ void wave_count_add(unsigned long long* ctr, unsigned v)
{
    for (int off = 32; off > 0; off >>= 1)
        v += __shfl_xor(v, off);
    if ((threadIdx.x & 63) == 0 && v)
        atomicAdd(ctr, (unsigned long long)v);
}

__device__ __forceinline__ uint32_t wave_append(unsigned int* counter, bool lead = true)
{
    const uint64_t m = __ballot(lead);
    const int leader = __ffsll((unsigned long long)m) - 1;
    uint32_t base = 0;
    if ((int)(threadIdx.x & 63) == leader)
        base = atomicAdd(counter, (unsigned)__popcll(m));
    base = __shfl(base, leader);
    return base + __builtin_amdgcn_mbcnt_hi((uint32_t)(m >> 32), __builtin_amdgcn_mbcnt_lo((uint32_t)m, 0u));
}

__device__ __forceinline__ float frame_roughness(const KParams& P, const Rec& h, const float* m)
{
    if (P.enable_roughness_mapping) {
// ... 1530 lines not shown
            break;
        if (tid == 0)
            s_next = 0;
        __syncthreads();
        for (int i = tid; i < n; i += 1024) {
            uint32_t out[rt::W_WIDTH];
            const int k = rt::wbvh_cut_expand(nodes, nnodes, cur[i], QS, out);
            const int base = atomicAdd(&s_next, k);
            for (int q = 0; q < k; q++)
                nxt[base + q] = out[q];
        }
        __syncthreads();
        if (tid == 0)
            s_n = s_next;
        uint32_t* t = cur;
        cur = nxt;
        nxt = t;
        __syncthreads();
    }
    const int n = s_n;
    if (cur != buf)
        for (int i = tid; i < n; i += 1024)
            buf[i] = cur[i];
    if (tid == 0)
        buf[2 * rt::W_CUT_MAX] = (uint32_t)n;
}

__global__ __launch_bounds__(256) void wide_mask_kernel(const rt::WNode* __restrict__ nodes, int nnodes,
                                                        const uint32_t* __restrict__ parent, const uint32_t* __restrict__ cut,
                                                        rt::WMaskCam C, uint32_t* words)
{
    const uint32_t i = blockIdx.x * 256u + threadIdx.x;
    if (i >= cut[2 * rt::W_CUT_MAX] || i >= (uint32_t)rt::W_CUT_MAX)
        return;
    const uint32_t en = cut[i];
    if ((int)(en >> 2) >= nnodes)
        return;
    rt::WMaskRect R = rt::wbvh_mask_entry(nodes, nnodes, parent, en, C);
    R.x0 = max(R.x0, 0);
    R.y0 = max(R.y0, 0);
    R.x1 = min(R.x1, C.bw - 1);
    R.y1 = min(R.y1, C.bh - 1);
    if (R.x0 > R.x1)
        return;
    for (int y = R.y0; y <= R.y1; y++)
        for (int w = R.x0 >> 5; w <= R.x1 >> 5; w++) {
            uint32_t* p = words + (size_t)y * C.wpr + w;
            const uint32_t m = rt::wbvh_mask_word(R, w);
            if ((__hip_atomic_load(p, __ATOMIC_RELAXED, __HIP_MEMORY_SCOPE_AGENT) & m) != m)
                atomicOr(p, m);
        }
}

hipError_t rt_launch_wide_cut(const rt::WNode* wnodes, int nnodes, int budget, int max_depth, uint32_t* buf, hipStream_t stream)
{
    budget = budget < rt::W_WIDTH ? rt::W_WIDTH : (budget > rt::W_CUT_MAX ? rt::W_CUT_MAX : budget);
    hipLaunchKernelGGL(wide_cut_kernel, dim3(1), dim3(1024), 0, stream, wnodes, nnodes, budget, max_depth, W_QS_CLOSEST, buf);
    return hipGetLastError();
}

hipError_t rt_launch_wide_mask(const rt::WNode* wnodes, int nnodes, const uint32_t* parent, const uint32_t* cut, int budget,
                               const rt::WMaskCam* C, uint32_t* words, hipStream_t stream)
{
    budget = budget < rt::W_WIDTH ? rt::W_WIDTH : (budget > rt::W_CUT_MAX ? rt::W_CUT_MAX : budget);
    hipError_t e = hipMemsetAsync(words, 0, (size_t)C->bh * C->wpr * 4, stream);
    if (e != hipSuccess)
        return e;
    hipLaunchKernelGGL(wide_mask_kernel, dim3((budget + 255) / 256), dim3(256), 0, stream, wnodes, nnodes, parent, cut,
                       *C, words);
    return hipGetLastError();
}

hipError_t rt_launch_wide_risk(const rt::GTri* wtris, const uint4* wmeta, const rt::GNode* onodes,
                               const rt::WNode* wnodes, const uint32_t* tri_leaf, const uint32_t* parent, uint32_t* K,
                               float* B, unsigned long long* risk, int n, int nnodes, const rt::WRiskArgs* A,
                               uint32_t* cap, const float* cap_dir, hipStream_t stream)
{
    rt::RiskCapDirs cd;
    for (int i = 0; i < 6; i++)
        cd.c[i / 3][i % 3] = cap_dir ? cap_dir[i] : 0.0f;
    if (n > 0)
        hipLaunchKernelGGL(rt::wide_risk_kernel, dim3((n + 255) / 256), dim3(256), 0, stream, wtris, wmeta, onodes,
                           tri_leaf, parent, K, B, n, *A, cap, cd);
    const int ne = 8 * nnodes;
    if (ne > 0)
        hipLaunchKernelGGL(rt::wide_risk_pack_kernel, dim3((ne + 255) / 256), dim3(256), 0, stream, wnodes, K, B, risk,
                           ne, *A);
    return hipGetLastError();
}

hipError_t rt_launch_wide_gather(const rt::GTri* tris, const int32_t* slot, const uint32_t* leaf_of_slot,
                                 const int32_t* tri_id, const int32_t* tri_mat, int n, rt::GTri* wtris, uint4* wmeta,
                                 hipStream_t stream)
{
    if (n <= 0)
        return hipSuccess;
    hipLaunchKernelGGL(rt::wide_gather_kernel, dim3((n + 255) / 256), dim3(256), 0, stream, tris, slot, leaf_of_slot,
                       tri_id, tri_mat, n, wtris, wmeta);
    return hipGetLastError();
}

namespace rt {
__global__ void ocone_fill_kernel(uint2* cells, size_t n)
{
    const size_t i = (size_t)blockIdx.x * 256 + threadIdx.x;
    if (i < n)
// ... 189 lines not shown
```

### raytracercpp_amd/csrc/kparams.hpp

```cpp
#pragma once

#include <stdint.h>

#include "octree.hpp"
#include "ocone.hpp"
#include "wbvh.hpp"

namespace rt {

#ifndef RT_SPLIT_G
#define RT_SPLIT_G 4
#endif
constexpr int SPLIT_G = RT_SPLIT_G;
constexpr int SPLIT_COLS = SPLIT_G == 8 ? 4 : 8;
constexpr int SPLIT_ROWS = 64 / SPLIT_G / SPLIT_COLS;
static_assert(SPLIT_G == 2 || SPLIT_G == 4 || SPLIT_G == 8, "2, 4 or 8 lanes per pixel");

constexpr int TEX_SLOTS = 6;
constexpr int MAT_STRIDE = 16;
constexpr int MAX_SHAPES = 64;
constexpr int NCOUNTERS = 32;
constexpr int TILE_SHARDS = 8;
constexpr int NCOUNTER_WORDS = NCOUNTERS + 16 * TILE_SHARDS;
constexpr int DBG_WAVES = 16384;
constexpr int DBG_WORDS = 8;

enum TexSlot { TEX_AO = 0, TEX_DIFFUSE = 1, TEX_NORMAL = 2, TEX_DISPLACEMENT = 3, TEX_ROUGHNESS = 4, TEX_SKYSPHERE = 5 };
enum Shading { RT_SHADING = 0, ABS_NORMALS = 1, PASTEL_NORMALS = 2, BARYCENTRIC = 3, VISUALIZE_AO = 4 };

struct KTex {
    const float4* px;
    int w, h;
};

struct KParams {
    const GNode* nodes;
    const GTri* tris;
    const int32_t* tri_id;
    const int32_t* tri_mat;
    const float* tri_uv;
    const float* cones;
    const float* lslab;
    float scene_scale;
    const float* lsin;
    const WNode* wnodes;
    const GTri* wtris;
    const uint4* wmeta;
    const uint64_t* wrisk;
    float risk_G, risk_nl, risk_nu;
    const float* risk_cap;
    float cap_dir[2][3];
    float sb_lo[3], sb_hi[3];
    int32_t sb_valid;
    const uint32_t* tile_mask;
    int32_t mask_wpr;
    OConeView ocone;
    int32_t nnodes;
    int32_t ntri_slots;
    int32_t levels;

    int32_t nshape;
    int32_t shape_kind[MAX_SHAPES];
    float shape[MAX_SHAPES][6];
    int32_t shape_mat[MAX_SHAPES];

    const float* mats;
    int32_t nmat;

    float cam_pos[3];
    float proj_inv[16];
    float cam_to_world[16];
    float light[3];
    int32_t proj_mode;
    float proj_w;
    int32_t c2w_affine;

    KTex tex[TEX_SLOTS];
    KTex sky[6];

    int32_t shading_method;
    int32_t compute_shadows;
    int32_t max_recursion_depth;
    int32_t enable_bvh;
    int32_t enable_ambient, enable_diffuse, enable_specular, enable_emissive;
    int32_t rough_reflections_sample_count;
    int32_t enable_ao_mapping, enable_diffuse_mapping, enable_normal_mapping, enable_displacement_mapping;
    float displacement_mapping_strength;
    int32_t parallax_mapping_steps;
    int32_t enable_roughness_mapping, enable_skysphere, enable_skybox;
    uint32_t rng_seed;
    int32_t has_reflection;
    float seg_scale;
    int32_t seg_oct;

    int32_t rw, rh;
    int32_t band_rows;
    int32_t nranks, rank;
    const int32_t* band_map;
    const int32_t* band_inv;
    int32_t local_rows;
    int32_t tiles_x, tiles_y;
    int32_t max_blocks;
    int32_t plain;
    uint32_t* tile_cost;
    unsigned long long* tile_stats;
    const int32_t* heavy_list;
    const uint32_t* heavy_bits;
    int32_t* heavy_ctr;
// ... 115 lines not shown
```

### raytracercpp_amd/csrc/launch.hpp

```cpp
#pragma once

#include <hip/hip_runtime.h>
#include <stdint.h>

#include "kparams.hpp"
#include "ocone.hpp"
#include "wbvh.hpp"

namespace rt {

enum class ReflStage {
    trace,
    long_,
    pass1,
    shadow,
    resolve,
};

enum class RasterStage {
    count,
    write,
    fill,
    fill_big,
};

}

#define RT_LAUNCH extern "C" __attribute__((visibility("hidden"))) hipError_t

RT_LAUNCH rt_launch_ray_trace(const rt::KParams* P, hipStream_t stream);
RT_LAUNCH rt_launch_heavy_prep(const rt::KParams* P, uint32_t* cost, int ntiles, int32_t* list, uint32_t* bits,
                               int32_t* ctr, int32_t* ctr_next, const unsigned long long* stats_prev,
                               unsigned long long* stats_next, float split, int group, hipStream_t stream);
RT_LAUNCH rt_launch_trace_rays(const rt::KParams* P, const float* o, const float* d, int n, int32_t* id, float* t,
                               float* u, float* v, uint8_t* ret, hipStream_t stream);
RT_LAUNCH rt_launch_wide_query(const rt::KParams* P, const float* o, const float* d, int n, int kind, float* o_out,
                               float* d_out, int32_t* status, int32_t* id, float* t, float* u, float* v, uint8_t* sh,
                               hipStream_t stream);
RT_LAUNCH rt_launch_trace_colors(const rt::KParams* P, bool refl, const float* o, const float* d, int n, float4* rgba,
                                 int32_t* src, float* t, uint8_t* found, uint8_t* shadow, hipStream_t stream);
RT_LAUNCH rt_launch_downscale(const uint32_t* in, int w, int h_rows, int f, uint32_t* out, hipStream_t stream);
RT_LAUNCH rt_launch_ssao(const rt::SsaoArgs* A, hipStream_t stream);

RT_LAUNCH rt_launch_wide_gather(const rt::GTri* tris, const int32_t* slot, const uint32_t* leaf_of_slot,
                                const int32_t* tri_id, const int32_t* tri_mat, int n, rt::GTri* wtris, uint4* wmeta,
                                hipStream_t stream);
RT_LAUNCH rt_launch_risk_box_init(float* B, size_t nentries, hipStream_t stream);
RT_LAUNCH rt_launch_wide_risk(const rt::GTri* wtris, const uint4* wmeta, const rt::GNode* onodes,
                              const rt::WNode* wnodes, const uint32_t* tri_leaf, const uint32_t* parent, uint32_t* K,
                              float* B, unsigned long long* risk, int n, int nnodes, const rt::WRiskArgs* A,
                              uint32_t* cap, const float* cap_dir, hipStream_t stream);
RT_LAUNCH rt_launch_wide_cut(const rt::WNode* wnodes, int nnodes, int budget, int max_depth, uint32_t* buf, hipStream_t stream);
RT_LAUNCH rt_launch_wide_mask(const rt::WNode* wnodes, int nnodes, const uint32_t* parent, const uint32_t* cut, int budget,
                              const rt::WMaskCam* C, uint32_t* words, hipStream_t stream);
RT_LAUNCH rt_launch_ocone(const rt::OConeEnt* E, const rt::GTri* tris, const uint32_t* todo, int n, const float lo[3],
                          const int32_t dim[3], double h, double r, double slack, double QS, double cos_cap,
                          uint2* cells, size_t ncells, hipStream_t stream);

RT_LAUNCH rt_launch_xform_points(const float m[16], float* pts, int64_t n, uint32_t* nonfinite, hipStream_t stream);
RT_LAUNCH rt_launch_gather_points(const float* verts, int64_t nv, const int32_t* idx, float* tri9, int64_t npts,
                                  uint32_t* flags, hipStream_t stream);

RT_LAUNCH rt_launch_refl_level0(const rt::KParams* P, rt::FrameRec* fr1, unsigned int* nfr1, hipStream_t stream);
RT_LAUNCH rt_launch_refl_stage(rt::ReflStage stage, const rt::KParams* P, const rt::ReflArgs* A, hipStream_t stream);
RT_LAUNCH rt_launch_refl_keys(const rt::KParams* P, const rt::FrameRec* fr, int n, uint32_t* keys, int32_t* idx,
                              hipStream_t stream);
RT_LAUNCH rt_launch_refl_sort_frames(const rt::FrameRec* fr, const int32_t* order, int n, rt::FrameRec* frs,
                                     hipStream_t stream);
RT_LAUNCH rt_launch_refl_shadow_keys(const rt::KParams* P, const rt::SampleRec* sm, const int32_t* list, int n,
                                     uint32_t* keys, hipStream_t stream);

RT_LAUNCH rt_launch_raster_stage(rt::RasterStage stage, const rt::KParams* P, const rt::RasterArgs* A, int npieces,
                                 hipStream_t stream);
RT_LAUNCH rt_launch_raster_shade(const rt::KParams* P, const rt::RasterArgs* A, rt::FrameRec* fr1, unsigned int* nfr1,
                                 hipStream_t stream);
```

### raytracercpp_amd/csrc/renderer.cpp

```cpp
#include "renderer.hpp"
#include "multidev.hpp"

#include <hipcub/hipcub.hpp>

#include <cstdlib>

#include <algorithm>
#include <chrono>
#include <cmath>
#include <cstring>
#include <thread>

#include "host_scene.hpp"
#include "launch.hpp"
#include "octree_gpu.hpp"
#include "wbvh_quick_gpu.hpp"

namespace rt {

DevBuf::~DevBuf() { release(); }

void DevBuf::release()
{
    if (p) {
// ... 46 lines not shown
static float ms_since(std::chrono::steady_clock::time_point t)
{
    return std::chrono::duration<float, std::milli>(std::chrono::steady_clock::now() - t).count();
}

Knobs Knobs::from_env()
{
    Knobs k;
    auto on = [](const char* name, bool dflt) {
        const char* v = getenv(name);
        return v ? v[0] != '0' : dflt;
    };
    auto flag = [](const char* name, bool dflt) {
        const char* v = getenv(name);
        return v ? atoi(v) != 0 : dflt;
    };
    auto num = [](const char* name, int dflt) {
        const char* v = getenv(name);
        return v ? atoi(v) : dflt;
    };
    auto real = [](const char* name, float dflt) {
        const char* v = getenv(name);
        return v ? (float)atof(v) : dflt;
    };
    k.wbvh = on("RT_WBVH", true);
    k.seg = on("RT_SEG", true);
    k.seg_oct = on("RT_SEG_OCTREE", false);
    k.cones = on("RT_CONES", true);
    k.lslab = on("RT_LSLAB", true);
    k.plain = on("RT_PLAIN", true);
    k.plain_octree = on("RT_PLAIN_OCTREE", true);
    k.quick_wbvh = on("RT_WBVH_QUICK_FIRST", true);
    k.fused_ssaa = on("RT_FUSED_SSAA", true);
    k.refl_engine = on("RT_REFL_ENGINE", true);
    k.debug_waves = getenv("RT_DEBUG_WAVES") != nullptr;
    k.exact = on("RT_EXACT", false);
    k.risk = on("RT_WBVH_RISK", true);
    k.heavy = on("RT_HEAVY_FIRST", true);
    if (getenv("RT_HEAVY_GROUP"))
        k.heavy_group = num("RT_HEAVY_GROUP", 0) > 1 ? SPLIT_G : 0;
    k.heavy_split = std::max(0.0f, real("RT_HEAVY_SPLIT", k.heavy_split));
    k.heavy_split_exp = std::max(0.0f, real("RT_HEAVY_SPLIT_EXP", k.heavy_split_exp));
    k.heavy_split_exp_overlap = std::max(0.0f, real("RT_HEAVY_SPLIT_EXP_OVERLAP", k.heavy_split_exp_overlap));
    if (getenv("RT_SPLIT_PARTS"))
        k.split_parts = num("RT_SPLIT_PARTS", 0) == 2 * SPLIT_G ? 2 * SPLIT_G : SPLIT_G;
    k.refl_defer = std::max(0, num("RT_REFL_DEFER", k.refl_defer));
    k.refl_feed = std::min(64, std::max(0, num("RT_REFL_FEED", k.refl_feed)));
    k.refl_sample_major = flag("RT_REFL_SAMPLE_MAJOR", k.refl_sample_major);
    k.refl_shadow_sort = flag("RT_REFL_SHADOW_SORT", k.refl_shadow_sort);
    k.refl_sorted_frames = flag("RT_REFL_SORTED_FRAMES", k.refl_sorted_frames);
    k.risk_cap = flag("RT_RISK_CAP", k.risk_cap);
    k.scene_bound = flag("RT_SCENE_BOUND", k.scene_bound);
    k.tile_mask = flag("RT_TILE_MASK", k.tile_mask);
    k.cut_budget = std::min((int)W_CUT_MAX, std::max((int)W_WIDTH, num("RT_TILE_MASK_CUT", k.cut_budget)));
    k.ocone = flag("RT_OCONE", k.ocone);
    k.ocone_dim = std::min(1024, std::max(1, num("RT_OCONE_DIM", k.ocone_dim)));
    k.inject_fail = num("RT_INJECT_FRAME_FAIL", 0);
    k.async_accel = on("RT_ASYNC_ACCEL", true);
    k.gpu_build = flag("RT_GPU_BUILD", k.gpu_build);
    k.gpu_xform = on("RT_GPU_XFORM", true);
    k.accel_hold = flag("RT_ACCEL_HOLD", k.accel_hold);
    k.accel_defer = flag("RT_ACCEL_DEFER", k.accel_defer);
    const int chunk = num("RT_REFL_CHUNK_LOG2", k.refl_chunk_log2);
    if (chunk >= 10 && chunk <= 27)
        k.refl_chunk_log2 = chunk;
    return k;
}

Renderer::Renderer(int device) : knobs_(Knobs::from_env()), device_(device)
{
    rt_default_settings(&s_);
    mat::identity(c2w_);
    mat::identity(w2c_);
    mat::identity(prev_object_);
    int rw, rh;
    render_size(rw, rh);
    img_w_ = rw;
    img_h_ = rh;
    aspect_ = (float)rw / rh;
    update_camera_projection();
}

int Renderer::init(std::string& err)
{
    hipError_t e = hipSetDevice(device_);
    if (e == hipSuccess)
        e = hipStreamCreateWithFlags(&stream_, hipStreamNonBlocking);
    if (e == hipSuccess)
        e = hipStreamCreateWithFlags(&accel_stream_, hipStreamNonBlocking);
    if (e == hipSuccess)
        e = hipStreamCreateWithFlags(&fence_stream_, hipStreamNonBlocking);
    if (e == hipSuccess)
        e = hipDeviceGetAttribute(&num_cus_, hipDeviceAttributeMultiprocessorCount, device_);
    for (int i = 0; i < 4 && e == hipSuccess; i++)
        e = hipEventCreate(&ev_[i]);
    if (e == hipSuccess)
        e = risk_fence_.create();
    if (e == hipSuccess)
        e = cut_fence_.create();
    if (e != hipSuccess) {
        err = std::string("HIP init failed: ") + hipGetErrorString(e);
        return RT_EHIP;
    }
    return RT_OK;
}

// ... 2248 lines not shown
    float cap_dir[2][3];
    for (int sel = 0; sel < 2; sel++) {
        const float* X = sel == 0 ? P.cam_pos : P.light;
        double v[3], l = 0;
        for (int a = 0; a < 3; a++) {
            v[a] = 0.5 * ((double)oct_root_.dn[a] + (double)oct_root_.df[a]) - (double)X[a];
            l += v[a] * v[a];
        }
        l = std::sqrt(l);
        for (int a = 0; a < 3; a++)
            cap_dir[sel][a] = l > 0 && l < INFINITY ? (float)(v[a] / l) : (a == 0 ? 1.0f : 0.0f);
    }
    hipError_t e;
    if (!risk_valid_ || std::memcmp(risk_cam_, P.cam_pos, sizeof risk_cam_) ||
        std::memcmp(risk_light_, P.light, sizeof risk_light_)) {
        if (wait_slots(stream) != RT_OK)
            return RT_EHIP;
        const float lo[3] = {oct_root_.dn[0], oct_root_.dn[1], oct_root_.dn[2]};
        const float hi[3] = {oct_root_.df[0], oct_root_.df[1], oct_root_.df[2]};
        const WRiskArgs A = wbvh_risk_args(lo, hi, P.scene_scale, P.cam_pos, P.light, W_QS_CLOSEST, W_QS_SHADOW);
        risk_valid_ = false;
        std::memcpy(risk_cap_dir_, cap_dir, sizeof risk_cap_dir_);
        if ((e = hipMemsetD32Async(reinterpret_cast<hipDeviceptr_t>(R.keys), 0x7F800000, R.entries, stream)) != hipSuccess ||
            (e = hipMemsetD32Async(reinterpret_cast<hipDeviceptr_t>(R.caps), 0x7F800000, 2, stream)) != hipSuccess ||
            (e = rt_launch_risk_box_init(R.boxes, R.entries, stream)) != hipSuccess ||
            (e = rt_launch_wide_risk(P.wtris, P.wmeta, P.nodes, P.wnodes, wide_.tri_leaf(), wide_.parent(), R.keys, R.boxes,
                                     R.words, (int)wide_.nt, (int)wide_.nn, &A, R.caps, &risk_cap_dir_[0][0], stream)) !=
                hipSuccess ||
            (e = risk_fence_.record(stream, fence_stream_)) != hipSuccess)
            return hip_fail(e, "wide_risk_kernel");
        risk_valid_ = true;
        std::memcpy(risk_cam_, P.cam_pos, sizeof risk_cam_);
        std::memcpy(risk_light_, P.light, sizeof risk_light_);
        risk_G_ = A.ray_G;
        risk_nl_ = A.ray_nl;
        risk_nu_ = A.ray_nu;
    } else if ((e = risk_fence_.wait_on(stream)) != hipSuccess)
        return hip_fail(e, "hipStreamWaitEvent (risk bits)");
    P.wrisk = reinterpret_cast<const uint64_t*>(R.words);
    P.risk_G = risk_G_;
    P.risk_nl = risk_nl_;
    P.risk_nu = risk_nu_;
    if (knobs_.risk_cap) {
        P.risk_cap = reinterpret_cast<const float*>(R.caps);
        std::memcpy(P.cap_dir, risk_cap_dir_, sizeof P.cap_dir);
    }
    return RT_OK;
}

int Renderer::prepare_mask(KParams& P, hipStream_t stream, MaskSlot& M)
{
    P.tile_mask = nullptr;
    P.mask_wpr = 0;
    mask_last_ = nullptr;
    mask_seen_ = true;
    if (!knobs_.tile_mask || !P.wnodes || !P.plain || P.has_reflection || P.zbuf || P.nbuf || wide_.nn <= 0 || !wide_.b_links.p ||
        s_.hybrid_rasterization_tracing)
        return RT_OK;
    const WMaskCam C = wbvh_mask_cam(P.proj_inv, P.cam_to_world, P.proj_mode, P.proj_w, P.c2w_affine, P.cam_pos, P.light,
                                     P.scene_scale, W_QS_CLOSEST, P.rw, P.rh);
    if (!C.valid)
        return RT_OK;
    hipError_t e;
    if (!cut_valid_) {
        if (wait_slots(stream) != RT_OK)
            return RT_EHIP;
        if ((e = d_cut_.reserve((size_t)(2 * W_CUT_MAX + 1) * 4)) != hipSuccess)
            return hip_fail(e, "hipMalloc (tile mask cut)");
        if ((e = rt_launch_wide_cut(P.wnodes, (int)wide_.nn, knobs_.cut_budget, W_CUT_DEPTH, d_cut_.as<uint32_t>(), stream)) !=
                hipSuccess ||
            (e = cut_fence_.record(stream, fence_stream_)) != hipSuccess)
            return hip_fail(e, "wide_cut_kernel");
        cut_valid_ = true;
        cut_gen_++;
    }
    if (M.cut_gen != cut_gen_ || std::memcmp(&C, &M.cam, sizeof C)) {
        M.cut_gen = 0;
        if ((e = M.words.reserve((size_t)C.bh * C.wpr * 4)) != hipSuccess)
            return hip_fail(e, "hipMalloc (tile mask)");
        if ((e = cut_fence_.wait_on(stream)) != hipSuccess ||
            (e = rt_launch_wide_mask(P.wnodes, (int)wide_.nn, wide_.parent(), d_cut_.as<uint32_t>(),
                                     knobs_.cut_budget, &C, M.words.as<uint32_t>(), stream)) != hipSuccess)
            return hip_fail(e, "wide_mask_kernel");
        M.cut_gen = cut_gen_;
        std::memcpy(&M.cam, &C, sizeof C);
    }
    P.tile_mask = M.words.as<uint32_t>();
    P.mask_wpr = C.wpr;
    mask_last_ = &M;
    return RT_OK;
}

int Renderer::prepare_heavy(KParams& P, TileCost& T, hipStream_t stream, uint64_t layout_key, bool* zeroed,
                            bool overlapped)
{
    if (zeroed)
        *zeroed = false;
    P.tile_cost = nullptr;
    P.heavy_list = nullptr;
    P.heavy_bits = nullptr;
    P.heavy_ctr = nullptr;
    P.heavy_group = 0;
    if (!knobs_.heavy || P.has_reflection || s_.hybrid_rasterization_tracing)
        return RT_OK;
    const int ntiles = P.tiles_x * P.tiles_y;
    if (ntiles <= 0)
        return RT_OK;
    const size_t nb = ((size_t)ntiles + 31) / 32;
    hipError_t e;
    const size_t stats_off = ((size_t)ntiles * 4 + nb * 4 + 7) / 8 * 8;
    if ((e = T.cost.reserve((size_t)ntiles * 4)) != hipSuccess ||
        (e = T.heavy.reserve(stats_off + 4 * 8 + 2 * 16)) != hipSuccess)
        return hip_fail(e, "hipMalloc (tile costs)");
    unsigned long long* stats = reinterpret_cast<unsigned long long*>(static_cast<char*>(T.heavy.p) + stats_off);
    int32_t* ctrs = reinterpret_cast<int32_t*>(stats + 4);
    uint64_t key = 1469598103934665603ull;
    for (int64_t v : {(int64_t)P.rw, (int64_t)P.rh, (int64_t)P.local_rows, (int64_t)P.tiles_x, (int64_t)P.tiles_y,
                      (int64_t)P.band_rows, (int64_t)P.rank, (int64_t)P.nranks, (int64_t)T.cost.bytes,
                      (int64_t)layout_key})
        key = (key ^ (uint64_t)v) * 1099511628211ull;
    if (key != T.key && ((e = hipMemsetAsync(T.cost.p, 0, (size_t)ntiles * 4, stream)) != hipSuccess ||
                         (e = hipMemsetAsync(stats, 0, 4 * 8 + 2 * 16, stream)) != hipSuccess))
        return hip_fail(e, "hipMemsetAsync (tile costs)");
    T.key = key;
    T.parity ^= 1u;
    T.ntiles = ntiles;
    T.tiles_x = P.tiles_x;
    T.tiles_y = P.tiles_y;
    int32_t* list = T.heavy.as<int32_t>();
    uint32_t* bits = reinterpret_cast<uint32_t*>(list + ntiles);
    int32_t* ctr = ctrs + 4 * T.parity;
    const int G = knobs_.heavy_group;
    const bool split = G > 1 && !P.has_reflection && P.plain && !P.zbuf && !P.nbuf && P.wnodes && P.nnodes > 0 &&
                       (!P.ds_out || ((1 << P.ds_shift) <= SPLIT_ROWS && (1 << P.ds_shift) <= SPLIT_COLS));
    unsigned long long* stats_next = stats + 2 * T.parity;
    const double share = (double)ntiles / (double)((int64_t)((P.rw + 7) / 8) * ((P.rh + 7) / 8));
    const float split_bar = knobs_.heavy_split *
                            (float)std::pow(std::min(1.0, std::max(share, 1e-6)),
                                            -(double)(overlapped ? knobs_.heavy_split_exp_overlap : knobs_.heavy_split_exp));
    if ((e = rt_launch_heavy_prep(&P, T.cost.as<uint32_t>(), ntiles, list, bits, ctr, ctrs + 4 * (T.parity ^ 1u),
                                  stats + 2 * (T.parity ^ 1u), stats_next, split_bar, split ? G : 0, stream)) != hipSuccess)
// ... 293 lines not shown
int Renderer::tile_mask(int src, uint32_t* out, int64_t cap, int32_t info[5])
{
    hipSetDevice(device_);
    if (!mask_seen_)
        return fail(RT_ESTATE, "tile_mask: no frame launch yet");
    if (src != 0 && src != 1)
        return fail(RT_EINVAL, "tile_mask: src is 0 (device) or 1 (host)");
    int rw, rh;
    render_size(rw, rh);
    const bool on = mask_last_ != nullptr;
    const int bw = on ? mask_last_->cam.bw : (rw + 7) / 8, bh = on ? mask_last_->cam.bh : (rh + 7) / 8, wpr = (bw + 31) / 32;
    info[0] = bw;
    info[1] = bh;
    info[2] = wpr;
    info[3] = on ? 1 : 0;
    info[4] = 0;
    const size_t nw = (size_t)bh * wpr;
    if (!out)
        return RT_OK;
    if (cap < (int64_t)nw)
        return fail(RT_EINVAL, "tile_mask: the buffer is too small");
    if (!on) {
        const WMaskRect all = {0, 0, bw - 1, bh - 1};
        for (int y = 0; y < bh; y++)
            for (int w = 0; w < wpr; w++)
                out[(size_t)y * wpr + w] = wbvh_mask_word(all, w);
        return RT_OK;
    }
    hipError_t e = hipDeviceSynchronize();
    uint32_t ncut = 0;
    if (e == hipSuccess)
        e = hipMemcpy(&ncut, d_cut_.as<uint32_t>() + 2 * W_CUT_MAX, 4, hipMemcpyDeviceToHost);
    if (e == hipSuccess && src == 0)
        e = hipMemcpy(out, mask_last_->words.p, nw * 4, hipMemcpyDeviceToHost);
    if (e != hipSuccess)
        return hip_fail(e, "tile_mask");
    info[4] = (int32_t)ncut;
    if (src == 1) {
        std::vector<WNode> nodes((size_t)wide_.nn);
        if ((e = hipMemcpy(nodes.data(), wide_.nodes(), nodes.size() * sizeof(WNode), hipMemcpyDeviceToHost)) != hipSuccess)
            return hip_fail(e, "download (wide BVH nodes)");
        std::vector<uint32_t> cut, words, parent(nodes.size());
        if ((e = hipMemcpy(parent.data(), wide_.parent(), parent.size() * 4, hipMemcpyDeviceToHost)) != hipSuccess)
            return hip_fail(e, "download (wide BVH parents)");
        wbvh_cut_host(nodes.data(), (int64_t)nodes.size(), knobs_.cut_budget, W_CUT_DEPTH, W_QS_CLOSEST, cut);
        wbvh_mask_host(nodes.data(), (int64_t)nodes.size(), parent.data(), cut, mask_last_->cam, words);
        if (cut.size() != ncut)
            return fail(RT_ESTATE, "tile_mask: the host's cut differs from the device's in size");
        std::memcpy(out, words.data(), nw * 4);
    }
    return RT_OK;
}

void Renderer::take_counters(const unsigned long long* cnt)
{
    last_shadow_ = (int64_t)cnt[0];
    last_refl_ = (int64_t)cnt[1];
    for (int i = 0; i < 4; i++) last_work_[i] = (int64_t)cnt[4 + i];
    for (int i = 0; i < 3; i++) last_work_[4 + i] = (int64_t)cnt[10 + i];
    last_work_[7] = (int64_t)cnt[14];
    for (int i = 0; i < 6; i++) last_uncert_[i] = (int64_t)cnt[16 + i];
    for (int i = 0; i < 6; i++) last_wave_[i] = (int64_t)cnt[22 + i];
}

float render(Renderer& renderer, int* rc)
{
    auto t0 = std::chrono::steady_clock::now();
    int r;
    if (renderer.multi_active() && !renderer.render_settings().enable_ssao) {
        r = renderer.render_multi();
    } else {
        r = renderer.render_settings().hybrid_rasterization_tracing ? renderer.raster_trace() : renderer.ray_trace();
        if (r == RT_OK)
            r = renderer.post_process();
    }
    if (rc)
        *rc = r;
    return std::chrono::duration<float, std::milli>(std::chrono::steady_clock::now() - t0).count();
}

}
```

### raytracercpp_amd/csrc/renderer.hpp

```cpp
#pragma once

#include <stdint.h>

#include <array>
#include <atomic>
#include <memory>
#include <mutex>
#include <string>
#include <thread>
#include <vector>

#include "../../include/rt_mi355x.h"
#include "kparams.hpp"
#include "ocone.hpp"
#include "octree.hpp"
#include "wbvh.hpp"
#include "wide_layout.hpp"

namespace rt {

struct OctreeGpuScratch;
struct OctreeDevInfo;
struct WQuickGpuScratch;

// ... 46 lines not shown
    }
    hipError_t record(hipStream_t stream, hipStream_t fence_stream)
    {
        hipError_t e;
        if ((e = hipEventRecord(mark_, stream)) == hipSuccess && (e = hipStreamWaitEvent(fence_stream, mark_, 0)) == hipSuccess &&
            (e = hipEventRecord(done_, fence_stream)) == hipSuccess)
            live_ = true;
        return e;
    }
    hipError_t wait_on(hipStream_t stream) const { return live_ ? hipStreamWaitEvent(stream, done_, 0) : hipSuccess; }
    hipError_t sync() const { return live_ ? hipEventSynchronize(done_) : hipSuccess; }
    bool live() const { return live_; }
    bool busy() const { return live_ && hipEventQuery(done_) == hipErrorNotReady; }

private:
    hipEvent_t mark_ = nullptr, done_ = nullptr;
    bool live_ = false;
};

struct HostTex {
    int w = 0, h = 0;
    std::vector<float> rgba;
};

struct Knobs {
    bool wbvh = true;
    bool seg = true;
    bool seg_oct = false;
    bool cones = true;
    bool lslab = true;
    bool plain = true;
    bool quick_wbvh = true;
    bool plain_octree = true;
    bool fused_ssaa = true;
    bool refl_engine = true;
    int refl_chunk_log2 = 27;
    bool debug_waves = false;
    bool exact = false;
    bool risk = true;
    bool heavy = true;
    int heavy_group = SPLIT_G;
    int split_parts = 0;
    float heavy_split_exp = 0.5f;
    float heavy_split_exp_overlap = 0.7f;
    float heavy_split = 0.5f;
    int refl_defer = 32;
    int refl_feed = 24;
    bool refl_sample_major = true;
    bool refl_shadow_sort = true;
    bool refl_sorted_frames = true;
    bool risk_cap = true;
    bool scene_bound = true;
    bool tile_mask = true;
    int cut_budget = W_CUT_BUDGET;
    bool ocone = true;
    int ocone_dim = 128;
    int inject_fail = 0;
    bool gpu_build = false;
    bool gpu_xform = true;
    bool async_accel = true;
    bool accel_hold = false;
    bool accel_defer = false;
    static Knobs from_env();
};

class Renderer {
public:
    explicit Renderer(int device);
    ~Renderer();
    int init(std::string& err);

    const rt_settings& render_settings() const { return s_; }
    int set_settings(const rt_settings& s);
    int set_exact(bool on);
    void set_device_build(bool on) { knobs_.gpu_build = on; }
    int64_t device_builds() const { return device_builds_; }
    int64_t device_wide_builds() const { return device_wide_builds_; }
    int64_t device_transforms() const { return device_xforms_; }
    int64_t device_ingests() const { return device_ingests_; }
    int64_t accel_builds() const { return accel_builds_; }
    void set_accel_deferred(bool on) { knobs_.accel_defer = on; }
    int set_triangles_device(const float* d_verts, int64_t nv, const int32_t* d_idx, const int32_t* mat,
                             const float* uv6, int64_t n, hipStream_t stream);
    int update_vertices_device(const float* d_verts, int64_t nv, const int32_t* d_idx, hipStream_t stream);
    int finish_accel();
    bool exact() const { return knobs_.exact; }
    int change_render_size(int w, int h);
    int set_triangles(const float* tri9, const int32_t* mat, const float* uv6, int64_t n);
    int add_sphere(float cx, float cy, float cz, float r, int mat);
    int add_plane(float px, float py, float pz, float nx, float ny, float nz, int mat);
    int clear_geometry();
    int set_materials(const float* mats16, int n);
    int material_count() const { return (int)(mats_.size() / MAT_STRIDE); }
    int change_camera_fov(float fov);
    int change_camera_aspect_ratio(float aspect);
    int set_light_position(float x, float y, float z);
    int set_camera_transform(const float m[16]);
    int apply_transformation_to_camera(const float m[16]);
    int set_camera_matrices(const float pos[3], const float proj_inv[16], const float c2w[16]);
    void get_camera_matrices(float pos[3], float proj_inv[16], float c2w[16]) const;
    int set_camera_projection(const float proj[16], const float w2c[16]);
    int set_camera_lens(float fov, float aspect);
    int set_object_transform(const float m[16]);
    int reset_previous_transform();
    int get_triangles(float* tri9, int64_t* n);
    int set_texture(int slot, int w, int h, const float* rgba);
    int set_skybox(const int32_t w[6], const int32_t h[6], const float* const faces[6]);
    int reconstruct_bvh_new();
    int destroy_bvh();
    int ray_trace();
    int raster_trace();
    int post_process();
    int get_image(uint32_t* argb, int32_t* w, int32_t* h);
    void lock_image() { image_mu_.lock(); }
    void unlock_image() { image_mu_.unlock(); }
    std::string display_error()
    {
        std::lock_guard<std::recursive_mutex> g(image_mu_);
        return display_err_;
    }
    int get_ssao_buffers(float* z, float* n4, int32_t* ao);
    int request_aux(bool rgba, bool hit, bool shadow);
    int get_internal(uint32_t* argb, float* rgba, int32_t* hit_id, float* hit_t, uint8_t* shadow);
    int get_stats(rt_stats* out) const;

    int local_rows(int band_rows, int rank, int nranks) const;
    int render_bands_device(int band_rows, int rank, int nranks, uint32_t* d_out, hipStream_t stream);
    int render_band_list_device(int band_rows, const int32_t* bands, int nbands, uint32_t* d_out, hipStream_t stream);
    int band_costs(hipStream_t stream, double* costs, int nbands);
    int kernel_times(float* ms, int n);
    int band_counters(unsigned long long out[2]);
    int tile_mask(int src, uint32_t* out, int64_t cap, int32_t info[5]);
    int debug_read(uint64_t* out, int64_t n);
    int tile_costs(uint32_t* out, int64_t n, int32_t* tiles_x, int32_t* tiles_y);
    int origin_cones(uint32_t* out, int64_t n, int32_t dims[3], float lo_ih[4]);
    int set_devices(const int* ids, int n);
    bool multi_active() const { return multi_ != nullptr; }
    int render_multi();

    int trace_rays(const float* orig, const float* dir, int64_t n, int32_t* id, float* t, float* u, float* v,
                   uint8_t* ret);
    int wide_query(const float* orig, const float* dir, int64_t n, int kind, float* o_out, float* d_out,
                   int32_t* status, int32_t* id, float* t, float* u, float* v, uint8_t* shadow);
    int risk_words(int src, uint64_t* out, int64_t cap, int64_t* count, int64_t* violations);
    int trace_ray_colors(const float* orig, const float* dir, int64_t n, int depth, float* rgba, int32_t* src,
                         float* t, uint8_t* found, uint8_t* shadow);

    const std::string& error() const { return err_; }

private:
    int fail(int code, const std::string& msg);
    int hip_fail(hipError_t e, const char* what);
    void render_size(int& w, int& h) const;
    void update_camera_projection();
    int ensure_device_scene();
    int rebuild_geometry();
    int build_octree(int64_t n, bool& dev_built);
    int upload_octree_tables(bool dev_built, hipError_t& e);
    int build_quick_wide(bool dev_built, hipError_t& e);
    int upload_materials();
    int upload_textures();
    int validate() const;
    void fill_params(KParams& P) const;
    int launch_trace(const KParams& P, hipStream_t stream);
    int launch_raster(const KParams& P, hipStream_t stream);
    int launch_frame(const KParams& P, hipStream_t stream)
    {
        return s_.hybrid_rasterization_tracing ? launch_raster(P, stream) : launch_trace(P, stream);
    }
    int check_frame() const;
    int launch_ssao();
    int trace_frame();
    int refl_level(const KParams& P, int level, int nframes, hipStream_t stream);
    int refl_level1_begin(const KParams& P, hipStream_t stream);
    int refl_level1_finish(const KParams& P, hipStream_t stream, const char* what, bool run_empty);
    static hipError_t read_u32(const void* dev, hipStream_t stream, unsigned& out);
    int wait_slots(hipStream_t stream);
    int sync_slots();

    Knobs knobs_;
    int device_;
    uint64_t geom_ver_ = 0, mats_ver_ = 0, tex_ver_ = 0;
    uint64_t mir_geom_ = ~0ull, mir_mats_ = ~0ull, mir_tex_ = ~0ull;
    std::thread accel_thread_;
    std::atomic<int> accel_state_{0};
// ... 66 lines not shown
    std::vector<int32_t> tri_mat_;
    int32_t tri_mat_lo_ = INT32_MAX, tri_mat_hi_ = INT32_MIN;
    std::vector<float> tri_uv_;
    std::vector<int32_t> shape_kind_;
    std::vector<float> shape_;
    std::vector<int32_t> shape_mat_;
    std::vector<float> mats_;
    float cam_pos_[3] = {0, 0, 0};
    float fov_ = 45.0f, near_ = 0.1f, far_ = 1000.0f, aspect_ = 1.0f;
    float proj_[16], proj_inv_[16], c2w_[16], w2c_[16];
    float light_[3] = {3, 3, 2};
    float prev_object_[16];
    HostTex tex_[TEX_SLOTS];
    HostTex sky_[6];
    bool has_bvh_ = false;

    FlatOctree oct_;
    int64_t oct_nn_ = 0, oct_nt_ = 0;
    int oct_levels_ = 0;
    GNode oct_root_{};
    OctreeStats oct_stats_{};
    bool has_uv_dev_ = false;
    bool geom_dirty_ = true, mats_dirty_ = true, tex_dirty_ = true;
    DevBuf d_nodes_, d_tris_, d_tri_id_, d_tri_mat_, d_tri_uv_, d_mats_;
    DevBuf d_tex_[TEX_SLOTS], d_sky_[6];
    DevBuf d_internal_, d_image_, d_rgba_, d_hit_id_, d_hit_t_, d_shadow_, d_counters_;
    DevBuf d_zbuf_, d_nbuf_, d_ao_;
    std::vector<float> cones_;
    DevBuf d_cones_;
    std::vector<float> lslab_;
    DevBuf d_lslab_;
    std::vector<float> lsin_;
    DevBuf d_lsin_;
    WBvh wb_;
    WideDev wide_;
    WBvh wb_next_;
    WideDev wide_next_;
    OConeGrid ocg_, ocg_next_;
    DevBuf d_ocone_, d_ocone2_, d_oc_ent_, d_oc_todo_;
    bool ocone_ready_ = false;
    float risk_cap_dir_[2][3] = {};
    hipError_t upload_wide(const WBvh& w, WideDev& d, hipStream_t stream);
    int reserve_risk(size_t nodes);
    DevBuf d_wrisk_;
    bool risk_valid_ = false;
    WNode sb_root_{};
    bool sb_root_valid_ = false;
    float risk_cam_[3] = {0, 0, 0}, risk_light_[3] = {0, 0, 0};
    float risk_G_ = 0.0f, risk_nl_ = 0.0f, risk_nu_ = 0.0f;
    Fence risk_fence_;
    int prepare_risk(KParams& P, hipStream_t stream);
    struct MaskSlot {
        DevBuf words;
        WMaskCam cam{};
        uint64_t cut_gen = 0;
    };
    DevBuf d_cut_;
    bool cut_valid_ = false, mask_seen_ = false;
    uint64_t cut_gen_ = 0;
    MaskSlot mask_main_;
    MaskSlot* mask_last_ = nullptr;
    Fence cut_fence_;
    int prepare_mask(KParams& P, hipStream_t stream, MaskSlot& M);
    DevBuf d_dbg_;
    bool ssao_ready_ = false;
    DevBuf d_tri9_, d_rcount_, d_roff_, d_pieces_, d_piece_uv_, d_zkey_, d_big_, d_scan_tmp_;
    bool want_rgba_ = false, want_hit_ = false, want_shadow_ = false;
    bool aux_valid_ = false;
    std::recursive_mutex image_mu_;
    hipStream_t display_stream_ = nullptr;
    hipEvent_t display_ev_[8] = {};
    void* display_host_ = nullptr;
    size_t display_bytes_ = 0;
    std::vector<void*> display_old_;
    int frames_started_ = 0;
    std::string display_err_;
    int begin_internal_image(int rw, int rh);
    int img_w_ = 0, img_h_ = 0;
    bool img_is_internal_ = false;
    bool rendered_ = false;

    struct ReflLevel {
        DevBuf fr, ret, sm, hit, cnt, list, sort, sort_tmp, res, frs, slist;
    };
    static constexpr int REFL_LEVELS = 18;
    ReflLevel refl_[REFL_LEVELS];

    struct TileCost {
        DevBuf cost, heavy;
        uint64_t key = 0;
        int ntiles = 0, tiles_x = 0, tiles_y = 0;
        uint32_t parity = 0;
        int band_rows = 0, ssaa = 1;
        std::vector<int32_t> bands;
    };
    int prepare_heavy(KParams& P, TileCost& T, hipStream_t stream, uint64_t layout_key = 0, bool* zeroed = nullptr,
                      bool overlapped = false);
    int render_bands_impl(int band_rows, int rank, int nranks, const int32_t* bands, int nbands, uint32_t* d_out,
                          hipStream_t stream);
    const TileCost* last_tc_ = nullptr;
    TileCost tc_main_;
    struct BandSlot {
        hipStream_t stream = nullptr;
        DevBuf counters, tmp;
        TileCost tc;
        Fence fence;
        DevBuf map;
        std::vector<int32_t> map_host;
        int map_nb = 0;
        uint64_t used = 0;
        MaskSlot mask;
    };
    static constexpr int BAND_SLOTS = 8;
    BandSlot band_slot_[BAND_SLOTS];
// ... 20 lines not shown
```

### raytracercpp_amd/csrc/wbvh.hpp

```cpp
#pragma once

#include <stdint.h>

#include <algorithm>
#include <cmath>
#include <vector>

#include "octree.hpp"

namespace rt {

constexpr uint32_t W_LEAF = 0x80000000u;
constexpr uint32_t W_EMPTY = 0xFFFFFFFFu;
constexpr int W_MAX_LEAF = 8;
#ifndef W_STACK_N
#define W_STACK_N 16
#endif
constexpr int W_STACK = W_STACK_N;
constexpr int W_WIDTH = 4;

#ifndef W_QS_CLOSEST
#define W_QS_CLOSEST 0x1p-10f
#endif
#ifndef W_QS_SHADOW
// ... 541 lines not shown
        const float* p = proj_inv + 4 * r;
        Tv[r] = std::fabs(pw) * (std::fabs((double)p[0]) + std::fabs((double)p[1]) + std::fabs((double)p[2]) + std::fabs((double)p[3]));
    }
    double vs[3][3];
    for (int r = 0; r < 3; r++) {
        const float* p = proj_inv + 4 * r;
        vs[r][0] = pw * (double)p[0] * ax;
        vs[r][1] = pw * (double)p[1] * ay;
        vs[r][2] = pw * ((double)p[0] * bx + (double)p[1] * by - (double)p[2] + (double)p[3]);
    }
    for (int r = 0; r < 3; r++) {
        const float* c = c2w + 4 * r;
        double Tw = std::fabs((double)c[3]) + std::fabs((double)cam[r]);
        for (int k = 0; k < 3; k++) {
            Tw += std::fabs((double)c[k]) * Tv[k];
            M[3 * r + k] = (double)c[0] * vs[0][k] + (double)c[1] * vs[1][k] + (double)c[2] * vs[2][k];
        }
        M[3 * r + 2] += (double)c[3] - (double)cam[r];
        T = std::max(T, Tw);
        C.cam[r] = cam[r];
    }
    const double c00 = M[4] * M[8] - M[5] * M[7], c01 = M[5] * M[6] - M[3] * M[8], c02 = M[3] * M[7] - M[4] * M[6];
    const double det = M[0] * c00 + M[1] * c01 + M[2] * c02;
    if (!std::isfinite(det) || !std::isfinite(T) || det == 0.0)
        return C;
    const double id = 1.0 / det;
    C.Minv[0] = c00 * id;
    C.Minv[1] = (M[2] * M[7] - M[1] * M[8]) * id;
    C.Minv[2] = (M[1] * M[5] - M[2] * M[4]) * id;
    C.Minv[3] = c01 * id;
    C.Minv[4] = (M[0] * M[8] - M[2] * M[6]) * id;
    C.Minv[5] = (M[2] * M[3] - M[0] * M[5]) * id;
    C.Minv[6] = c02 * id;
    C.Minv[7] = (M[1] * M[6] - M[0] * M[7]) * id;
    C.Minv[8] = (M[0] * M[4] - M[1] * M[3]) * id;
    double rn[3], res = 0.0;
    for (int r = 0; r < 3; r++) {
        rn[r] = std::sqrt(C.Minv[3 * r] * C.Minv[3 * r] + C.Minv[3 * r + 1] * C.Minv[3 * r + 1] + C.Minv[3 * r + 2] * C.Minv[3 * r + 2]);
        for (int k = 0; k < 3; k++) {
            const double x = C.Minv[3 * r] * M[k] + C.Minv[3 * r + 1] * M[3 + k] + C.Minv[3 * r + 2] * M[6 + k];
            res = std::max(res, std::fabs(x - (r == k ? 1.0 : 0.0)));
        }
    }
    const double E = 0x1p-18 * T;
    const double ds = rn[2] * E;
    const double shift = 2.0 * (std::max(rn[0], rn[1]) * E + std::max(rw, rh) * ds);
    if (!(res < 1e-9) || !(ds <= 0.5) || !(shift <= 1.0))
        return C;
    C.guard = guard_override ? *guard_override : 1.0 + 4.0 * shift;
    C.valid = 1;
    return C;
}

struct WMaskRect {
    int32_t x0, y0, x1, y1;
};

RT_HD WMaskRect wbvh_mask_rect(const WNode& N, int j, const WMaskCam& C)
{
    const WMaskRect all = {0, 0, C.bw - 1, C.bh - 1};
    const WBoundCtx B = wbvh_bound_ctx(N, C.cam, C.light_finite != 0, C.S);
    if (!B.valid)
        return all;
    double W = wbvh_child_reach(N, j, B, C.QS);
    if (W < 0.0)
        return all;
    W = (W + 1.125 * (double)B.m) * (1.0 + 0x1p-19);
    double lo[3], hi[3];
    for (int a = 0; a < 3; a++) {
        const double l = (double)B.org[a] + (double)N.qlo[a][j] * (double)B.st[a] - W;
        const double h = (double)B.org[a] + (double)N.qhi[a][j] * (double)B.st[a] + W;
        const double c = 0.5 * (l + h), r = 0.5 * (h - l) * C.scale;
        lo[a] = c - r - (double)C.cam[a];
        hi[a] = c + r - (double)C.cam[a];
        if (!(fabs(lo[a]) < 0x1p27) || !(fabs(hi[a]) < 0x1p27) || !(lo[a] <= hi[a]))
            return all;
    }
    double xmin = INFINITY, xmax = -INFINITY, ymin = INFINITY, ymax = -INFINITY, smin = INFINITY, smax = -INFINITY;
    for (int c = 0; c < 8; c++) {
        const double px = (c & 1) ? hi[0] : lo[0], py = (c & 2) ? hi[1] : lo[1], pz = (c & 4) ? hi[2] : lo[2];
        const double a = C.Minv[0] * px + C.Minv[1] * py + C.Minv[2] * pz;
        const double b = C.Minv[3] * px + C.Minv[4] * py + C.Minv[5] * pz;
        const double s = C.Minv[6] * px + C.Minv[7] * py + C.Minv[8] * pz;
        smin = fmin(smin, s);
        smax = fmax(smax, s);
        const double x = a / s, y = b / s;
        xmin = fmin(xmin, x);
        xmax = fmax(xmax, x);
        ymin = fmin(ymin, y);
        ymax = fmax(ymax, y);
    }
    const double sa = fmax(fabs(smin), fabs(smax));
    if (!(smin * smax > 0.0) || !(fmin(fabs(smin), fabs(smax)) > 0x1p-20 * sa) || !(sa < INFINITY))
        return all;
    xmin -= C.guard;
    xmax += C.guard;
    ymin -= C.guard;
    ymax += C.guard;
    if (!(xmin <= xmax) || !(ymin <= ymax))
        return WMaskRect{1, 1, 0, 0};
    if (xmax < 0.0 || ymax < 0.0 || xmin > (double)(C.rw - 1) || ymin > (double)(C.rh - 1))
        return WMaskRect{1, 1, 0, 0};
    WMaskRect R;
    R.x0 = (int32_t)floor(fmax(xmin, 0.0)) >> 3;
    R.y0 = (int32_t)floor(fmax(ymin, 0.0)) >> 3;
    R.x1 = (int32_t)ceil(fmin(xmax, (double)(C.rw - 1))) >> 3;
    R.y1 = (int32_t)ceil(fmin(ymax, (double)(C.rh - 1))) >> 3;
    return R;
}

RT_HD WMaskRect wbvh_mask_entry(const WNode* nodes, int64_t nnodes, const uint32_t* parent, uint32_t entry, const WMaskCam& C)
{
    WMaskRect R = wbvh_mask_rect(nodes[entry >> 2], (int)(entry & 3u), C);
    uint32_t n = entry >> 2;
    for (int up = 0; parent && up < 64 && R.x0 <= R.x1 && R.y0 <= R.y1; up++) {
        const uint32_t p = parent[n];
        if (p == W_EMPTY || (int64_t)(p >> 2) >= nnodes)
            break;
        const WMaskRect Q = wbvh_mask_rect(nodes[p >> 2], (int)(p & 3u), C);
        R.x0 = R.x0 > Q.x0 ? R.x0 : Q.x0;
        R.y0 = R.y0 > Q.y0 ? R.y0 : Q.y0;
        R.x1 = R.x1 < Q.x1 ? R.x1 : Q.x1;
        R.y1 = R.y1 < Q.y1 ? R.y1 : Q.y1;
        n = p >> 2;
    }
    if (R.x0 > R.x1 || R.y0 > R.y1)
        return WMaskRect{1, 1, 0, 0};
    return R;
}

RT_HD uint32_t wbvh_mask_word(const WMaskRect& R, int w)
{
    const int b0 = R.x0 - 32 * w, b1 = R.x1 - 32 * w;
    if (b1 < 0 || b0 > 31)
        return 0u;
    const uint32_t lo = b0 <= 0 ? 0xFFFFFFFFu : 0xFFFFFFFFu << b0;
    const uint32_t hi = b1 >= 31 ? 0xFFFFFFFFu : 0xFFFFFFFFu >> (31 - b1);
    return lo & hi;
}

inline void wbvh_mask_host(const WNode* nodes, int64_t nnodes, const uint32_t* parent, const std::vector<uint32_t>& cut,
                           const WMaskCam& C, std::vector<uint32_t>& words)
{
    words.assign((size_t)C.bh * C.wpr, 0u);
    for (uint32_t en : cut) {
        const WMaskRect R = wbvh_mask_entry(nodes, nnodes, parent, en, C);
        for (int y = R.y0; y <= R.y1 && R.x0 <= R.x1; y++)
            for (int w = R.x0 >> 5; w <= R.x1 >> 5; w++)
                words[(size_t)y * C.wpr + w] |= wbvh_mask_word(R, w);
    }
}

struct WRiskArgs {
    double p[2][3];
    double G[2], nu[2], slack[2], QS[2];
    int32_t on[2];
    float ray_G, ray_nl, ray_nu;
};

inline WRiskArgs wbvh_risk_args(const float lo[3], const float hi[3], float S, const float cam[3], const float light[3],
                                float qs_cam, float qs_light)
{
    WRiskArgs A{};
    double cm = 0, lm = 0, gc = 0;
    for (int a = 0; a < 3; a++) {
        A.p[0][a] = cam[a];
        A.p[1][a] = light[a];
        cm = std::max(cm, std::fabs((double)cam[a]));
        lm = std::max(lm, std::fabs((double)light[a]));
    }
    for (int c = 0; c < 8; c++) {
        double g = 0;
        for (int a = 0; a < 3; a++) {
            const double x = ((c >> a) & 1) ? hi[a] : lo[a];
            g += (x - light[a]) * (x - light[a]);
        }
        gc = std::max(gc, std::sqrt(g));
    }
    A.ray_nl = 2.0f;
    const double G = 1.01 * (gc + 1e-4 * A.ray_nl) + 0x1p-10 * (S + lm);
    A.ray_G = std::nextafter((float)G, 0.0f);
    A.G[0] = 0.0;
    A.nu[0] = 0.0;
    A.slack[0] = 1.01 * 0x1p-16 * (cm + S);
    A.QS[0] = qs_cam;
    A.G[1] = G;
    A.nu[1] = 1.001e-4 * A.ray_nl + 16.0 * 0x1p-24 * G;
    A.ray_nu = std::nextafter((float)(A.nu[1] * (1 + 1e-6)), INFINITY);
    A.slack[1] = 1.01 * 0x1p-16 * (lm + G + S);
    A.QS[1] = qs_light;
    const bool fin = std::isfinite(cm) && std::isfinite(lm) && std::isfinite(G);
    A.on[0] = A.on[1] = fin ? 1 : 0;
    return A;
}

RT_HD bool risk_cap_skip(float s, const float c[3], v3 d, float QS)
{
    const float dl = sqrtf(d.x * d.x + d.y * d.y + d.z * d.z);
    const float cg = fabsf(c[0] * d.x + c[1] * d.y + c[2] * d.z) / dl;
    const float x = c[1] * d.z - c[2] * d.y, y = c[2] * d.x - c[0] * d.z, z = c[0] * d.y - c[1] * d.x;
    const float sg = sqrtf(x * x + y * y + z * z) / dl;
    return s * cg - sqrtf(fmaxf(0.0f, 1.0f - s * s)) * sg >= QS + 0x1p-14f;
}
// ... 136 lines not shown
#if defined(__HIP_DEVICE_COMPILE__)
    if constexpr (G <= 4) {
        x = fminf(x, __uint_as_float(wg_quad<0xB1>(__float_as_uint(x))));
        if (G == 4)
            x = fminf(x, __uint_as_float(wg_quad<0x4E>(__float_as_uint(x))));
    } else {
        for (int m = 1; m < G; m <<= 1)
            x = fminf(x, __shfl_xor(x, m));
    }
#endif
    return x;
}
template <int G, class T>
RT_HD T wg_read(T x, int i)
{
    static_assert(sizeof(T) == 4, "32-bit values");
#if defined(__HIP_DEVICE_COMPILE__)
    if constexpr (G <= 4) {
        uint32_t u;
        __builtin_memcpy(&u, &x, 4);
        uint32_t r;
        if (G == 4) {
            const uint32_t b0 = wg_quad<0x00>(u), b1 = wg_quad<0x55>(u), b2 = wg_quad<0xAA>(u), b3 = wg_quad<0xFF>(u);
            r = i == 0 ? b0 : i == 1 ? b1 : i == 2 ? b2 : b3;
        } else {
            const uint32_t b0 = wg_quad<0xA0>(u), b1 = wg_quad<0xF5>(u);
            r = i == 0 ? b0 : b1;
        }
        T y;
        __builtin_memcpy(&y, &r, 4);
        return y;
    } else {
        return __shfl(x, (int)(__lane_id() & ~(uint32_t)(G - 1)) + i);
    }
#else
    (void)i;
    return x;
#endif
}

struct WNoFeed {
    static constexpr bool on = false;
    bool busy = false;
    bool drained = true;
    int threshold = 64;
    template <class H> RT_HD void finish(int, H&, v3, v3) {}
    RT_HD bool fetch(bool, v3&, v3&, float&, bool&) { return false; }
};

template <class Stack, int G = 1, class Feed = WNoFeed>
RT_HD int wbvh_closest(const WNode* nodes, const GTri* tris, v3 o, v3 d, float m, Stack& stk, WHit& h,
                       uint32_t* work = nullptr, float hi = INFINITY, bool ties = true, float QS = 0x1p-8f,
                       const uint64_t* risk = nullptr, int rsel = 0, float rsub = 0.0f, uint32_t max_steps = 0,
                       Feed* feed = nullptr, bool nob = false)
{
    static_assert(G == 1 || ((G & (G - 1)) == 0 && G <= 8 && (Stack::CAP & (Stack::CAP - 1)) == 0),
                  "a lane group: a power of two up to 8 lanes, a ring stack of 2^k entries");
    constexpr bool FEED = Feed::on;
    static_assert(!FEED || G == 1, "lane refill: one lane per query");
    auto slot = [](int i) { return G > 1 ? (i & (Stack::CAP - 1)) : i; };
    h.t = INFINITY;
    h.u = 1.0f;
    h.v = 0.0f;
    h.k = -1;
    const float DMIN = 0x1p-100f;
    constexpr float SL = 0x1p-20f;
    constexpr float NLH = 127.9f;
    float ix, iy, iz, aix, aiy, aiz, dl, cstep, idl, icp, iqd;
    bool nx_lo, ny_lo, nz_lo;
    auto setup = [&]() {
        ix = 1.0f / (fabsf(d.x) < DMIN ? copysignf(DMIN, d.x) : d.x);
        iy = 1.0f / (fabsf(d.y) < DMIN ? copysignf(DMIN, d.y) : d.y);
        iz = 1.0f / (fabsf(d.z) < DMIN ? copysignf(DMIN, d.z) : d.z);
        nx_lo = !(ix < 0.0f);
        ny_lo = !(iy < 0.0f);
        nz_lo = !(iz < 0.0f);
        aix = fabsf(ix);
        aiy = fabsf(iy);
        aiz = fabsf(iz);
        dl = sqrtf(d.x * d.x + d.y * d.y + d.z * d.z) * (1.0f + 0x1p-20f);
        cstep = dl * W_CONE_STEP;
        idl = fast_rcp(sqrtf(d.x * d.x + d.y * d.y + d.z * d.z) * (1.0f - 0x1p-20f)) * (1.0f + 0x1p-18f);
        icp = (1.0f - 0x1p-18f) / (NLH * dl);
        iqd = (1.0f - 0x1p-20f) / (QS * dl);
    };
    setup();
    float best_s = hi + fabsf(hi) * SL;
    bool tie = false, nanhit = false, infhit = false;
    float dropped = INFINITY;
    int sp = 0, bot = 0;
    uint32_t cur = FEED || (G > 1 && wg_lane<G>() != 0) ? W_EMPTY : 0u;
    uint32_t nn = 0, nt = 0;
    uint32_t steps = 0;
    auto status = [&]() -> int {
        const bool ovf = dropped < INFINITY && dropped <= best_s;
        if (nanhit)
            return W_UNCERT;
        if (h.k < 0) {
            if (infhit)
                return W_UNCERT;
            if (ovf)
                return W_DEEP;
            h.t = -1.0f;
            return W_MISS;
        }
        if ((ties && tie) || !(h.t > 0.0f && h.t < INFINITY))
            return W_UNCERT;
        return ovf ? W_DEEP : W_HIT;
    };
    (void)status;
    auto refill = [&]() -> bool {
        if constexpr (FEED) {
#if defined(__HIP_DEVICE_COMPILE__)
            const bool idle_lane = cur == W_EMPTY;
            const uint64_t idle = __ballot(idle_lane);
            if (idle != 0ull && (idle == __ballot(1) || __popcll(idle) >= feed->threshold)) {
                if (idle_lane && feed->busy)
                    feed->finish(status(), h, o, d);
                if (feed->fetch(idle_lane, o, d, m, nob)) {
                    setup();
                    h.t = INFINITY;
                    h.u = 1.0f;
                    h.v = 0.0f;
                    h.k = -1;
                    best_s = hi + fabsf(hi) * SL;
                    tie = nanhit = infhit = false;
                    dropped = INFINITY;
                    sp = bot = 0;
                    cur = 0u;
                }
                return __ballot(cur != W_EMPTY) != 0ull || !feed->drained;
            }
#endif
        }
        return true;
    };
    while (FEED ? refill() : (G > 1 ? wg_bits<G>(cur != W_EMPTY) != 0u : cur != W_EMPTY)) {
        if constexpr (FEED) {
            if (cur == W_EMPTY)
                continue;
        }
        ++steps;
        if (max_steps && steps > max_steps)
            return W_LONG;
// ... 315 lines not shown
```

### raytracercpp_amd/renderer.py

```python
from __future__ import annotations

import ctypes as C
import time
from typing import Optional, Sequence

import numpy as np

from . import _lib
from ._lib import RtSettings, RtStats, check, f32, ptr
from .scene import RenderSettings, SceneData, SHAPE_SPHERE, TEX_AO, TEX_DIFFUSE, TEX_NORMAL, TEX_DISPLACEMENT, \
    TEX_ROUGHNESS, TEX_SKYSPHERE

_f32p = C.POINTER(C.c_float)
_i32p = C.POINTER(C.c_int32)
_u32p = C.POINTER(C.c_uint32)
_u8p = C.POINTER(C.c_uint8)


def _to_c(st: RenderSettings) -> RtSettings:
    c = RtSettings()
    _lib.lib().rt_default_settings(C.byref(c))
    for name, typ in RtSettings._fields_:
        if hasattr(st, name):
            v = getattr(st, name)
# ... 335 lines not shown
        d = f32(dirs).reshape(-1, 3)
        if d.shape != o.shape:
            raise ValueError(f"wide_query: {o.shape[0]} origins but {d.shape[0]} directions")
        n = o.shape[0]
        out = dict(o=np.zeros((n, 3), np.float32), d=np.zeros((n, 3), np.float32), status=np.zeros(n, np.int32),
                   id=np.zeros(n, np.int32), t=np.zeros(n, np.float32), u=np.zeros(n, np.float32),
                   v=np.zeros(n, np.float32), shadowed=np.zeros(n, np.uint8))
        self._call("rt_wide_query", ptr(o, _f32p), ptr(d, _f32p), n, int(kind), ptr(out["o"], _f32p),
                   ptr(out["d"], _f32p), ptr(out["status"], _i32p), ptr(out["id"], _i32p), ptr(out["t"], _f32p),
                   ptr(out["u"], _f32p), ptr(out["v"], _f32p), ptr(out["shadowed"], _u8p))
        return out

    def risk_words(self, src=0):
        n, bad = C.c_int64(), C.c_int64()
        self._call("rt_risk_words", int(src), None, 0, C.byref(n), None)
        out = np.zeros(n.value, np.uint64)
        self._call("rt_risk_words", int(src), out.ctypes.data_as(C.POINTER(C.c_uint64)), out.size, C.byref(n),
                   C.byref(bad))
        return out, bad.value

    def trace_ray(self, orig, dirs, current_recursion_depth=0):
        o = f32(orig).reshape(-1, 3)
        d = f32(dirs).reshape(-1, 3)
        if d.shape != o.shape:
            raise ValueError(f"trace_ray: {o.shape[0]} origins but {d.shape[0]} directions")
        n = o.shape[0]
        rgba = np.zeros((n, 4), np.float32)
        src = np.zeros(n, np.int32)
        t = np.zeros(n, np.float32)
        found = np.zeros(n, np.uint8)
        shadowed = np.zeros(n, np.uint8)
        self._call("rt_trace_ray", ptr(o, _f32p), ptr(d, _f32p), n, int(current_recursion_depth), ptr(rgba, _f32p),
                   ptr(src, _i32p), ptr(t, _f32p), ptr(found, _u8p), ptr(shadowed, _u8p))
        return rgba, src, t, found, shadowed

    def kernel_times(self, n):
        ms = np.zeros(n, np.float32)
        self._call("rt_kernel_times", ptr(ms, _f32p), int(n))
        return ms

    def band_counters(self):
        a, b = C.c_int64(), C.c_int64()
        self._call("rt_band_counters", C.byref(a), C.byref(b))
        return a.value, b.value

    def tile_mask(self, src=0):
        info = np.zeros(5, np.int32)
        self._call("rt_tile_mask", int(src), None, 0, ptr(info, _i32p))
        bw, bh, wpr = int(info[0]), int(info[1]), int(info[2])
        words = np.zeros(bh * wpr, np.uint32)
        self._call("rt_tile_mask", int(src), ptr(words, _u32p), words.size, ptr(info, _i32p))
        bits = (words.reshape(bh, wpr)[:, :, None] >> np.arange(32, dtype=np.uint32)) & 1
        return bits.reshape(bh, wpr * 32)[:, :bw].astype(bool), {"on": bool(info[3]), "cut": int(info[4])}

    def load_scene(self, sc: SceneData, st: RenderSettings):
        self.set_render_settings(st)
        self.change_render_size(st.image_width, st.image_height)
        self.set_camera_matrices(sc.cam_pos, sc.proj_inv, sc.cam_to_world)
        if sc.proj is not None and sc.world_to_cam is not None:
            self.set_camera_projection(sc.proj, sc.world_to_cam)
        self.set_camera_lens(*sc.lens(st))
        self.set_light_position(sc.light)
        self.set_materials(sc.materials)
        self.clear_geometry()
        for k in range(len(sc.shape_kind)):
            s = sc.shape[k]
            if sc.shape_kind[k] == SHAPE_SPHERE:
                self.add_sphere(s[:3], s[3], int(sc.shape_mat[k]))
            else:
                self.add_plane(s[:3], s[3:6], int(sc.shape_mat[k]))
        self.set_triangles(sc.tri, sc.tri_mat, sc.tri_uv)
        for slot in range(6):
            self._set_tex(slot, sc.textures.get(slot) if sc.textures else None)
        if sc.skybox is not None:
            self.set_skybox(sc.skybox)


def render(renderer: Renderer) -> float:
    ms = C.c_float()
    check(_lib.lib().rt_render(renderer._h, C.byref(ms)), "rt_render")
    return float(ms.value)
```

Baseline: 9770 Mrays/s.

## Start wide-BVH primary traversal from per-8x8-tile entry node sets

Computes, for each 8x8 screen tile, up to four wide-BVH nodes whose projected bounds cover the tile, found by descending from the root and sorted by distance to the camera. Primary rays in the plain wide path then begin traversal at these entry nodes instead of the root, with the extra entries pushed onto the stack. This is meant to skip the upper-level node visits that every ray in a tile would otherwise repeat. It adds a per-tile start table (built and uploaded per mask update), one uint4 load per ray, and relies on the projected-rect test being conservative for correctness. It also adds probe and diagnostic APIs.

Measured after the change: 10390 Mrays/s, median of 6. +6.3%, better.

```diff
diff --git a/__graft_entry__.py b/__graft_entry__.py
--- a/__graft_entry__.py
+++ b/__graft_entry__.py
@@ -26,6 +26,8 @@
     build_program()
     from tile_mask_tool import build_program as build_tile_mask_program
     build_tile_mask_program()
+    from tile_starts_tool import build_program as build_tile_starts_program
+    build_tile_starts_program()
     if os.path.isdir("/root/reference/tp2"):
         from test_reference_adapter import build_adapter_program
         build_adapter_program()
diff --git a/include/rt_mi355x.h b/include/rt_mi355x.h
--- a/include/rt_mi355x.h
+++ b/include/rt_mi355x.h
@@ -190,6 +190,7 @@
 int rt_kernel_times(rt_renderer *r, float *ms, int32_t n);
 int rt_band_counters(rt_renderer *r, int64_t *shadow_rays, int64_t *reflection_rays);
 int rt_tile_mask(rt_renderer *r, int32_t src, uint32_t *words, int64_t cap, int32_t info[5]);
+int rt_tile_starts(rt_renderer *r, int32_t src, uint32_t *sets, int64_t cap, int32_t info[3]);
 
 void rt_make_transform(int32_t kind, float x, float y, float z, float out[16]);
 void rt_compose(const float a[16], const float b[16], float out[16]);
diff --git a/include/rt_mi355x_diag.h b/include/rt_mi355x_diag.h
--- a/include/rt_mi355x_diag.h
+++ b/include/rt_mi355x_diag.h
@@ -20,10 +20,21 @@
 int rt_wbvh_query(const float *tri9, int64_t n, int32_t max_depth, int32_t leaf_max_obj_count, const float *orig,
                   const float *dir, int64_t nrays, int32_t *status, int32_t *id, float *t, float *u, float *v,
                   int64_t stats[8], float *ms);
+typedef struct rt_entry_probe {
+    float proj_inv[16], cam_to_world[16];
+    int32_t rw, rh;
+    int32_t k, fan, depth;
+    int32_t quick;
+    const int32_t *pixel;
+    uint32_t *sets;
+    int64_t info[4];
+    int64_t depth_hist[16];
+} rt_entry_probe;
 int rt_wbvh_query_ex(const float *tri9, int64_t n, int32_t max_depth, int32_t leaf_max_obj_count, const float *orig,
                      const float *dir, int64_t nrays, const float *cam, const float *light, int32_t shadow_rays,
                      float *o_out, float *d_out, int32_t *status, int32_t *id, float *t, float *u, float *v,
-                     int64_t stats[8], float *ms, int32_t *ray_nodes, int32_t ocone_dim, int64_t oc_stats[5]);
+                     int64_t stats[8], float *ms, int32_t *ray_nodes, int32_t ocone_dim, int64_t oc_stats[5],
+                     rt_entry_probe *entry);
 
 int rt_ocone_check(const float *tri9, int64_t n, int32_t max_depth, int32_t leaf_max_obj_count, int32_t ocone_dim,
                    const float *orig, const float *dir, int64_t nrays, int32_t *skip, int64_t out[6],
diff --git a/raytracercpp_amd/_lib.py b/raytracercpp_amd/_lib.py
--- a/raytracercpp_amd/_lib.py
+++ b/raytracercpp_amd/_lib.py
@@ -61,6 +61,14 @@
                 return [float(x) if n == "build_split_ms" else int(x) for x in v]
             return int(v)
         return {n: conv(n, t) for n, t in self._fields_}
+
+
+class RtEntryProbe(C.Structure):
+    _fields_ = [
+        ("proj_inv", C.c_float * 16), ("cam_to_world", C.c_float * 16), ("rw", C.c_int32), ("rh", C.c_int32),
+        ("k", C.c_int32), ("fan", C.c_int32), ("depth", C.c_int32), ("quick", C.c_int32),
+        ("pixel", _i32p), ("sets", _u32p), ("info", C.c_int64 * 4), ("depth_hist", C.c_int64 * 16),
+    ]
 
 
 _H = C.c_void_p
@@ -128,6 +136,7 @@
     "rt_kernel_times": (C.c_int, [_H, _f32p, C.c_int32]),
     "rt_band_counters": (C.c_int, [_H, _i64p, _i64p]),
     "rt_tile_mask": (C.c_int, [_H, C.c_int32, _u32p, C.c_int64, _i32p]),
+    "rt_tile_starts": (C.c_int, [_H, C.c_int32, _u32p, C.c_int64, _i32p]),
     "rt_make_transform": (None, [C.c_int32, C.c_float, C.c_float, C.c_float, _f32p]),
     "rt_compose": (None, [_f32p, _f32p, _f32p]),
     "rt_inverse": (None, [_f32p, _f32p]),
@@ -153,7 +162,7 @@
                                 _f32p, _f32p, _i64p, _f32p]),
     "rt_wbvh_query_ex": (C.c_int, [_f32p, C.c_int64, C.c_int32, C.c_int32, _f32p, _f32p, C.c_int64, _f32p, _f32p,
                                    C.c_int32, _f32p, _f32p, _i32p, _i32p, _f32p, _f32p, _f32p, _i64p, _f32p, _i32p,
-                                   C.c_int32, _i64p]),
+                                   C.c_int32, _i64p, C.POINTER(RtEntryProbe)]),
     "rt_ocone_check": (C.c_int, [_f32p, C.c_int64, C.c_int32, C.c_int32, C.c_int32, _f32p, _f32p, C.c_int64, _i32p,
                                  _i64p, C.POINTER(C.c_uint32), _i32p, _f32p, C.POINTER(C.c_uint32)]),
     "rt_ocone_read": (C.c_int, [_H, C.POINTER(C.c_uint32), C.c_int64, _i32p, _f32p]),
@@ -336,7 +345,7 @@
 
 
 def wbvh_query(tri9, orig, dirs, max_depth=12, leaf=40, cam=None, light=None, shadow_rays=False, rays_out=False,
-               ray_nodes=None, ocone_dim=0, oc_stats=None):
+               ray_nodes=None, ocone_dim=0, oc_stats=None, entry=None):
     tri9 = f32(tri9).reshape(-1, 9)
     o = f32(orig).reshape(-1, 3)
     d = f32(dirs).reshape(-1, 3)
@@ -350,13 +359,29 @@
     do = np.zeros((n, 3), np.float32)
     c = None if cam is None else f32(cam).reshape(3)
     li = None if light is None else f32(light).reshape(3)
+    ep = None
+    if entry is not None:
+        ep = RtEntryProbe()
+        ep.proj_inv[:] = [float(x) for x in f32(entry["proj_inv"]).ravel()]
+        ep.cam_to_world[:] = [float(x) for x in f32(entry["cam_to_world"]).ravel()]
+        ep.rw, ep.rh = int(entry["rw"]), int(entry["rh"])
+        ep.k, ep.fan, ep.depth = (int(entry.get(x, 0)) for x in ("k", "fan", "depth"))
+        ep.quick = int(entry.get("quick", 0))
+        pix = np.ascontiguousarray(entry["pixel"], np.int32).reshape(-1, 2)
+        assert pix.shape[0] == n
+        sets = np.zeros(((ep.rh + 7) // 8, (ep.rw + 7) // 8, 4), np.uint32)
+        ep.pixel = ptr(pix, _i32p)
+        ep.sets = ptr(sets, _u32p)
     check(lib().rt_wbvh_query_ex(ptr(tri9, _f32p), tri9.shape[0], max_depth, leaf, ptr(o, _f32p), ptr(d, _f32p), n,
                                  None if c is None else ptr(c, _f32p), None if li is None else ptr(li, _f32p),
                                  1 if shadow_rays else 0, ptr(oo, _f32p), ptr(do, _f32p),
                                  ptr(st, _i32p), ptr(ids, _i32p), ptr(t, _f32p), ptr(u, _f32p), ptr(v, _f32p),
                                  ptr(stats, _i64p), ptr(ms, _f32p),
                                  None if ray_nodes is None else ptr(ray_nodes, _i32p), int(ocone_dim),
-                                 None if oc_stats is None else ptr(oc_stats, _i64p)), "rt_wbvh_query")
+                                 None if oc_stats is None else ptr(oc_stats, _i64p),
+                                 None if ep is None else C.byref(ep)), "rt_wbvh_query")
+    if ep is not None:
+        entry.update(sets=sets, has_mask=bool(ep.info[2]), covered=int(ep.info[3]), depth_hist=[int(x) for x in ep.depth_hist])
     keys = ("nodes", "leaves", "max_leaf", "depth", "node_visits", "tri_tests", "violations", "sah_x1000")
     out = (st, ids, t, u, v, dict(zip(keys, map(int, stats))), (float(ms[0]), float(ms[1])))
     return out + (oo, do) if rays_out else out
diff --git a/raytracercpp_amd/csrc/capi.cpp b/raytracercpp_amd/csrc/capi.cpp
--- a/raytracercpp_amd/csrc/capi.cpp
+++ b/raytracercpp_amd/csrc/capi.cpp
@@ -472,6 +472,10 @@
 int rt_tile_mask(rt_renderer* r, int32_t src, uint32_t* words, int64_t cap, int32_t info[5])
 {
     return guarded(R(r), [&] { return info ? R(r)->tile_mask(src, words, cap, info) : RT_EINVAL; });
+}
+int rt_tile_starts(rt_renderer* r, int32_t src, uint32_t* sets, int64_t cap, int32_t info[3])
+{
+    return guarded(R(r), [&] { return info ? R(r)->tile_starts(src, sets, cap, info) : RT_EINVAL; });
 }
 int rt_band_counters(rt_renderer* r, int64_t* shadow_rays, int64_t* reflection_rays)
 {
@@ -1196,16 +1200,17 @@
                   int64_t stats[8], float* ms)
 {
     return rt_wbvh_query_ex(tri9, n, max_depth, leaf_max_obj_count, orig, dir, nrays, nullptr, nullptr, 0, nullptr,
-                            nullptr, status, id, t, u, v, stats, ms, nullptr, 0, nullptr);
+                            nullptr, status, id, t, u, v, stats, ms, nullptr, 0, nullptr, nullptr);
 }
 
 int rt_wbvh_query_ex(const float* tri9, int64_t n, int32_t max_depth, int32_t leaf_max_obj_count, const float* orig,
                      const float* dir, int64_t nrays, const float* cam, const float* light, int32_t shadow_rays,
                      float* o_out, float* d_out, int32_t* status, int32_t* id, float* t, float* u, float* v,
-                     int64_t stats[8], float* ms, int32_t* ray_nodes, int32_t ocone_dim, int64_t oc_stats[5])
+                     int64_t stats[8], float* ms, int32_t* ray_nodes, int32_t ocone_dim, int64_t oc_stats[5],
+                     rt_entry_probe* entry)
 {
     if (n < 0 || (n > 0 && !tri9) || nrays < 0 || (nrays > 0 && (!orig || !dir || !status || !id || !t || !u || !v)) ||
-        (shadow_rays && !light))
+        (shadow_rays && !light) || (entry && (!cam || shadow_rays || (nrays > 0 && !entry->pixel) || entry->rw <= 0 || entry->rh <= 0)))
         return bad("rt_wbvh_query: bad arguments");
     try {
         rt::FlatOctree f;
@@ -1213,7 +1218,10 @@
         auto t0 = std::chrono::steady_clock::now();
         rt::build_flat_octree(tri9, n, max_depth, leaf_max_obj_count, f);
         auto t1 = std::chrono::steady_clock::now();
-        rt::build_wbvh(f, w);
+        if (entry && entry->quick)
+            rt::build_wbvh_quick(f, w);
+        else
+            rt::build_wbvh(f, w);
         if (ms) {
             ms[0] = std::chrono::duration<float, std::milli>(t1 - t0).count();
             ms[1] = std::chrono::duration<float, std::milli>(std::chrono::steady_clock::now() - t1).count();
@@ -1279,6 +1287,47 @@
                 }
                 ocv.ih = ocg.ih;
             }
+        }
+        std::vector<uint32_t> esets;
+        int ebw = 0;
+        if (entry) {
+            int mode;
+            float pw;
+            rt::wbvh_proj_shortcut(entry->proj_inv, mode, pw);
+            const float* c = entry->cam_to_world;
+            const int affine = c[12] == 0.0f && c[13] == 0.0f && c[14] == 0.0f && c[15] == 1.0f;
+            const rt::WMaskCam C = rt::wbvh_mask_cam(entry->proj_inv, c, mode, pw, affine, cam, light, S, W_QS_CLOSEST,
+                                                     entry->rw, entry->rh);
+            entry->info[0] = C.bw;
+            entry->info[1] = C.bh;
+            entry->info[2] = usable && C.valid;
+            entry->info[3] = 0;
+            if (usable && C.valid) {
+                std::vector<uint32_t> cut, words;
+                rt::wbvh_cut_host(w.nodes.data(), (int64_t)w.nodes.size(), W_CUT_BUDGET, W_CUT_DEPTH, W_QS_CLOSEST, cut);
+                rt::wbvh_mask_host(w.nodes.data(), (int64_t)w.nodes.size(), w.parent.data(), cut, C, words);
+                for (uint32_t x : words)
+                    entry->info[3] += __builtin_popcount(x);
+                rt::wbvh_entry_host(w.nodes.data(), (int64_t)w.nodes.size(), C, words.data(), entry->k > 0 ? entry->k : W_ENTRY_K,
+                                    entry->fan > 0 ? entry->fan : W_ENTRY_FAN, entry->depth > 0 ? entry->depth : W_CUT_DEPTH,
+                                    esets);
+                ebw = C.bw;
+            }
+            if (entry->sets) {
+                const size_t nb = (size_t)C.bw * C.bh;
+                for (size_t b = 0; b < nb; b++)
+                    for (int k = 0; k < rt::W_ENTRY_MAX; k++)
+                        entry->sets[b * rt::W_ENTRY_MAX + k] = esets.empty() ? (k ? rt::W_EMPTY : 0u) : esets[b * rt::W_ENTRY_MAX + k];
+            }
+            for (int k = 0; k < 16; k++)
+                entry->depth_hist[k] = 0;
+            for (uint32_t l : esets)
+                if (l != rt::W_EMPTY && l != 0u) {
+                    int dep = 0;
+                    for (uint32_t x = l; dep < 15 && w.parent[x] != rt::W_EMPTY; x = w.parent[x] >> 2)
+                        dep++;
+                    entry->depth_hist[dep]++;
+                }
         }
         std::atomic<int64_t> work_n{0}, work_t{0}, n_nob{0};
         const bool probe_hi = std::getenv("RT_WQ_PROBE_HI") != nullptr;
@@ -1343,9 +1392,15 @@
                     nob = rt::risk_cap_skip(cap[1], cap_dir[1], d, W_QS_SHADOW);
                 if (nob)
                     ++n_nob;
+                const uint32_t* start = nullptr;
+                if (!esets.empty() && rk) {
+                    const int px = entry->pixel[2 * i], py = entry->pixel[2 * i + 1];
+                    if (px >= 0 && py >= 0 && px < entry->rw && py < entry->rh)
+                        start = &esets[((size_t)(py >> 3) * ebw + (px >> 3)) * rt::W_ENTRY_MAX];
+                }
                 int st = rt::wbvh_closest(w.nodes.data(), w.tris.data(), o, d, m, stk, h, wk, INFINITY, true,
                                           shadow_rays ? W_QS_SHADOW : W_QS_CLOSEST, rk, rsel, rsub, 0u,
-                                          (rt::WNoFeed*)nullptr, nob);
+                                          (rt::WNoFeed*)nullptr, nob, start);
                 if (st == rt::W_DEEP) {
                     rt::WStackArr<rt::W_DEEP_STACK> deep;
                     st = rt::wbvh_closest(w.nodes.data(), w.tris.data(), o, d, m, deep, h, wk, INFINITY, true,
diff --git a/raytracercpp_amd/csrc/kernels.hip b/raytracercpp_amd/csrc/kernels.hip
--- a/raytracercpp_amd/csrc/kernels.hip
+++ b/raytracercpp_amd/csrc/kernels.hip
@@ -814,7 +814,8 @@
 
 template <class Stk, int G>
 __device__ __forceinline__ int wide_run(const KParams& P, v3 o, v3 d, uint2* lv, WHit& w, float hi, bool ties, float QS,
-                                        const uint64_t* rk, int rsel, float rsub, uint32_t max_steps, bool nob, int count)
+                                        const uint64_t* rk, int rsel, float rsub, uint32_t max_steps, bool nob, int count,
+                                        const uint32_t* start = nullptr)
 {
     const float m = wide_margin(P, o);
     Stk stk{lv};
@@ -825,7 +826,7 @@
     uint32_t* wk = nullptr;
 #endif
     int st = wbvh_closest<Stk, G>(P.wnodes, P.wtris, o, d, m, stk, w, wk, hi, ties, QS, rk, rsel, rsub, max_steps,
-                                  (WNoFeed*)nullptr, nob);
+                                  (WNoFeed*)nullptr, nob, start);
 #if RT_COUNT
     if (wk) {
         count_wave_steps(P, count, wk[3]);
@@ -852,9 +853,9 @@
     return kdop_certifies(load_gnode(P.nodes + M.y), o, d, w.t);
 }
 
-template <int G = 1, int CAP = W_STACK>
+template <int G = 1, int CAP = W_STACK, bool START = false>
 __device__ __forceinline__ bool wide_closest(const KParams& P, v3 o, v3 d, THit& h, bool& r, uint2* lv,
-                                             Rec* rec = nullptr, uint32_t max_steps = 0, bool* longq = nullptr)
+                                             Rec* rec = nullptr, uint32_t max_steps = 0, bool* longq = nullptr, int bidx = -1)
 {
     using Stk = WStackLdsN<G == 1 ? CAP : W_STACK>;
     WHit w;
@@ -862,8 +863,17 @@
     const uint64_t* rk = P.wrisk && cam ? P.wrisk : nullptr;
     const bool nob = rk && P.risk_cap && risk_cap_skip(P.risk_cap[0], P.cap_dir[0], d, W_QS_CLOSEST);
     int st = W_MISS;
-    if (!(cam && P.sb_valid && scene_bound_rejects(P.sb_lo, P.sb_hi, o, d)))
-        st = wide_run<Stk, G>(P, o, d, lv, w, INFINITY, true, W_QS_CLOSEST, rk, 0, 0.0f, RT_COUNT ? 0u : max_steps, nob, 22);
+    if (!(cam && P.sb_valid && scene_bound_rejects(P.sb_lo, P.sb_hi, o, d))) {
+        if constexpr (START) {
+            uint32_t s[W_ENTRY_MAX] = {0u, W_EMPTY, W_EMPTY, W_EMPTY};
+            if (bidx >= 0 && cam) {
+                const uint4 e = ldg(P.tile_start + bidx);
+                s[0] = e.x; s[1] = e.y; s[2] = e.z; s[3] = e.w;
+            }
+            st = wide_run<Stk, G>(P, o, d, lv, w, INFINITY, true, W_QS_CLOSEST, rk, 0, 0.0f, RT_COUNT ? 0u : max_steps, nob, 22, s);
+        } else
+            st = wide_run<Stk, G>(P, o, d, lv, w, INFINITY, true, W_QS_CLOSEST, rk, 0, 0.0f, RT_COUNT ? 0u : max_steps, nob, 22);
+    }
     if (max_steps && st == W_LONG) {
         *longq = true;
         return false;
@@ -1087,7 +1097,7 @@
 }
 
 template <bool PLAIN = false, int G = 1, bool OCT = false>
-__device__ int closest_hit(const KParams& P, v3 o, v3 d, Rec& fin, uint2* lv)
+__device__ int closest_hit(const KParams& P, v3 o, v3 d, Rec& fin, uint2* lv, int bidx = -1)
 {
     Rec local = rec_fresh();
     int src = -1;
@@ -1095,7 +1105,7 @@
         THit h;
         bool r = false;
         const bool wide = !OCT && P.wnodes && P.nnodes > 0 && !ray_is_nan(o, d);
-        if (wide && wide_closest<G, PLAIN ? W_STACK_PLAIN : W_STACK>(P, o, d, h, r, lv, &local)) {
+        if (wide && wide_closest<G, PLAIN ? W_STACK_PLAIN : W_STACK, PLAIN && !OCT>(P, o, d, h, r, lv, &local, 0u, nullptr, bidx)) {
             if (r && (local.t < fin.t || fin.t == -1)) {
                 fin = local;
                 src = local.tri;
@@ -1321,13 +1331,13 @@
 
 template <bool REFL, bool PLAIN = false, int G = 1, bool OCT = false>
 __device__ PixelOut trace_pixel(const KParams& P, v3 cam, v3 rd0, uint2* lv, uint32_t pixel_key, unsigned& nshadow,
-                                unsigned& nrefl)
+                                unsigned& nrefl, int bidx = -1)
 {
     PixelOut po;
     po.fin = rec_fresh();
     po.found = po.shadowed = false;
     po.alpha = 1.0f;
-    po.src = closest_hit<PLAIN && !REFL, REFL ? 1 : G, OCT>(P, cam, rd0, po.fin, lv);
+    po.src = closest_hit<PLAIN && !REFL, REFL ? 1 : G, OCT>(P, cam, rd0, po.fin, lv, bidx);
     if (PLAIN) PH_MARK(2);
     if (!REFL) {
         if (PLAIN && po.fin.t > 0.1f) {
@@ -1707,6 +1717,11 @@
     return normalize(ws - cam);
 }
 
+__device__ __forceinline__ int tile_start_index(const KParams& P, int px, int py)
+{
+    return P.tile_start ? (py >> 3) * P.start_bw + (px >> 3) : -1;
+}
+
 template <int G>
 __device__ __forceinline__ void trace_split_part(const KParams& P, uint2* lv, int t, int lane, unsigned& nshadow)
 {
@@ -1729,7 +1744,7 @@
         const v3 cam = mk(P.cam_pos[0], P.cam_pos[1], P.cam_pos[2]);
         const v3 rd = camera_dir(P, px, py, cam);
         unsigned ns = 0, nr = 0;
-        PixelOut po = trace_pixel<false, true, G>(P, cam, rd, lv, 0u, ns, nr);
+        PixelOut po = trace_pixel<false, true, G>(P, cam, rd, lv, 0u, ns, nr, tile_start_index(P, px, py));
         if ((lane & (G - 1)) == 0)
             nshadow += ns;
         const size_t o = (size_t)lr * P.rw + px;
@@ -1850,7 +1865,8 @@
         if (PLAIN) PH_MARK(1);
 
         uint32_t rng = REFL ? pixel_seed((uint32_t)(py * P.rw + px), P.rng_seed) : 0u;
-        PixelOut po = trace_pixel<REFL, PLAIN, 1, OCT>(P, cam, rd, lv, rng, nshadow, nrefl);
+        PixelOut po = trace_pixel<REFL, PLAIN, 1, OCT>(P, cam, rd, lv, rng, nshadow, nrefl,
+                                                        PLAIN && !REFL && !OCT ? tile_start_index(P, px, py) : -1);
         size_t o = (size_t)lr * P.rw + px;
         if (P.argb) P.argb[o] = color_to_argb(po.color);
         if (!REFL && P.ds_out) downscale_tile(P, lane, lr, px, color_to_argb(po.color));
@@ -3487,6 +3503,33 @@
         }
 }
 
+__global__ __launch_bounds__(256) void wide_entry_kernel(const rt::WNode* __restrict__ nodes, int nnodes, rt::WMaskCam C,
+                                                         const uint32_t* __restrict__ words, int K, int fan, int max_depth,
+                                                         uint4* out)
+{
+    const uint32_t i = blockIdx.x * 256u + threadIdx.x;
+    if (i >= (uint32_t)(C.bw * C.bh))
+        return;
+    const int bx = (int)(i % (uint32_t)C.bw), by = (int)(i / (uint32_t)C.bw);
+    uint4 r = make_uint4(0u, rt::W_EMPTY, rt::W_EMPTY, rt::W_EMPTY);
+    if ((words[(size_t)by * C.wpr + (bx >> 5)] >> (bx & 31)) & 1u) {
+        const rt::WEntrySet S = rt::wbvh_entry_block(nodes, nnodes, C, bx, by, K, fan, max_depth);
+        r = make_uint4(S.link[0], S.link[1], S.link[2], S.link[3]);
+    }
+    out[i] = r;
+}
+
+hipError_t rt_launch_wide_entry(const rt::WNode* wnodes, int nnodes, const rt::WMaskCam* C, const uint32_t* words, int K,
+                                int fan, int max_depth, uint4* out, hipStream_t stream)
+{
+    const int nb = C->bw * C->bh;
+    if (nb <= 0)
+        return hipSuccess;
+    hipLaunchKernelGGL(wide_entry_kernel, dim3((nb + 255) / 256), dim3(256), 0, stream, wnodes, nnodes, *C, words, K, fan,
+                       max_depth, out);
+    return hipGetLastError();
+}
+
 hipError_t rt_launch_wide_cut(const rt::WNode* wnodes, int nnodes, int budget, int max_depth, uint32_t* buf, hipStream_t stream)
 {
     budget = budget < rt::W_WIDTH ? rt::W_WIDTH : (budget > rt::W_CUT_MAX ? rt::W_CUT_MAX : budget);
diff --git a/raytracercpp_amd/csrc/kparams.hpp b/raytracercpp_amd/csrc/kparams.hpp
--- a/raytracercpp_amd/csrc/kparams.hpp
+++ b/raytracercpp_amd/csrc/kparams.hpp
@@ -54,6 +54,8 @@
     int32_t sb_valid;
     const uint32_t* tile_mask;
     int32_t mask_wpr;
+    const uint4* tile_start;
+    int32_t start_bw;
     OConeView ocone;
     int32_t nnodes;
     int32_t ntri_slots;
diff --git a/raytracercpp_amd/csrc/launch.hpp b/raytracercpp_amd/csrc/launch.hpp
--- a/raytracercpp_amd/csrc/launch.hpp
+++ b/raytracercpp_amd/csrc/launch.hpp
@@ -53,6 +53,8 @@
 RT_LAUNCH rt_launch_wide_cut(const rt::WNode* wnodes, int nnodes, int budget, int max_depth, uint32_t* buf, hipStream_t stream);
 RT_LAUNCH rt_launch_wide_mask(const rt::WNode* wnodes, int nnodes, const uint32_t* parent, const uint32_t* cut, int budget,
                               const rt::WMaskCam* C, uint32_t* words, hipStream_t stream);
+RT_LAUNCH rt_launch_wide_entry(const rt::WNode* wnodes, int nnodes, const rt::WMaskCam* C, const uint32_t* words, int K,
+                               int fan, int max_depth, uint4* out, hipStream_t stream);
 RT_LAUNCH rt_launch_ocone(const rt::OConeEnt* E, const rt::GTri* tris, const uint32_t* todo, int n, const float lo[3],
                           const int32_t dim[3], double h, double r, double slack, double QS, double cos_cap,
                           uint2* cells, size_t ncells, hipStream_t stream);
diff --git a/raytracercpp_amd/csrc/renderer.cpp b/raytracercpp_amd/csrc/renderer.cpp
--- a/raytracercpp_amd/csrc/renderer.cpp
+++ b/raytracercpp_amd/csrc/renderer.cpp
@@ -122,6 +122,7 @@
     k.risk_cap = flag("RT_RISK_CAP", k.risk_cap);
     k.scene_bound = flag("RT_SCENE_BOUND", k.scene_bound);
     k.tile_mask = flag("RT_TILE_MASK", k.tile_mask);
+    k.tile_start = flag("RT_TILE_START", k.tile_start);
     k.cut_budget = std::min((int)W_CUT_MAX, std::max((int)W_WIDTH, num("RT_TILE_MASK_CUT", k.cut_budget)));
     k.ocone = flag("RT_OCONE", k.ocone);
     k.ocone_dim = std::min(1024, std::max(1, num("RT_OCONE_DIM", k.ocone_dim)));
@@ -2476,7 +2477,10 @@
 {
     P.tile_mask = nullptr;
     P.mask_wpr = 0;
+    P.tile_start = nullptr;
+    P.start_bw = 0;
     mask_last_ = nullptr;
+    starts_last_ = false;
     mask_seen_ = true;
     if (!knobs_.tile_mask || !P.wnodes || !P.plain || P.has_reflection || P.zbuf || P.nbuf || wide_.nn <= 0 || !wide_.b_links.p ||
         s_.hybrid_rasterization_tracing)
@@ -2508,9 +2512,25 @@
             return hip_fail(e, "wide_mask_kernel");
         M.cut_gen = cut_gen_;
         std::memcpy(&M.cam, &C, sizeof C);
+        M.starts_valid = false;
+        M.launches = 0;
+    }
+    M.launches++;
+    if (knobs_.tile_start && !M.starts_valid && M.launches >= 2) {
+        if ((e = M.starts.reserve((size_t)C.bh * C.bw * sizeof(uint4))) != hipSuccess)
+            return hip_fail(e, "hipMalloc (entry sets)");
+        if ((e = rt_launch_wide_entry(P.wnodes, (int)wide_.nn, &C, M.words.as<uint32_t>(), W_ENTRY_K, W_ENTRY_FAN,
+                                      W_CUT_DEPTH, M.starts.as<uint4>(), stream)) != hipSuccess)
+            return hip_fail(e, "wide_entry_kernel");
+        M.starts_valid = true;
     }
     P.tile_mask = M.words.as<uint32_t>();
     P.mask_wpr = C.wpr;
+    if (M.starts_valid) {
+        P.tile_start = M.starts.as<uint4>();
+        P.start_bw = C.bw;
+        starts_last_ = true;
+    }
     mask_last_ = &M;
     return RT_OK;
 }
@@ -2910,6 +2930,48 @@
     return RT_OK;
 }
 
+int Renderer::tile_starts(int src, uint32_t* out, int64_t cap, int32_t info[3])
+{
+    hipSetDevice(device_);
+    if (!mask_seen_)
+        return fail(RT_ESTATE, "tile_starts: no frame launch yet");
+    if (src != 0 && src != 1)
+        return fail(RT_EINVAL, "tile_starts: src is 0 (device) or 1 (host)");
+    int rw, rh;
+    render_size(rw, rh);
+    const bool on = mask_last_ != nullptr && starts_last_;
+    const int bw = mask_last_ ? mask_last_->cam.bw : (rw + 7) / 8, bh = mask_last_ ? mask_last_->cam.bh : (rh + 7) / 8;
+    info[0] = bw;
+    info[1] = bh;
+    info[2] = on ? 1 : 0;
+    const size_t nw = (size_t)bw * bh * W_ENTRY_MAX;
+    if (!out)
+        return RT_OK;
+    if (cap < (int64_t)nw)
+        return fail(RT_EINVAL, "tile_starts: the buffer is too small");
+    if (!on) {
+        for (size_t i = 0; i < nw; i++)
+            out[i] = i % W_ENTRY_MAX ? W_EMPTY : 0u;
+        return RT_OK;
+    }
+    hipError_t e = hipDeviceSynchronize();
+    if (e == hipSuccess && src == 0)
+        e = hipMemcpy(out, mask_last_->starts.p, nw * 4, hipMemcpyDeviceToHost);
+    if (e != hipSuccess)
+        return hip_fail(e, "tile_starts");
+    if (src == 1) {
+        const WMaskCam& C = mask_last_->cam;
+        std::vector<WNode> nodes((size_t)wide_.nn);
+        std::vector<uint32_t> words((size_t)C.bh * C.wpr), sets;
+        if ((e = hipMemcpy(nodes.data(), wide_.nodes(), nodes.size() * sizeof(WNode), hipMemcpyDeviceToHost)) != hipSuccess ||
+            (e = hipMemcpy(words.data(), mask_last_->words.p, words.size() * 4, hipMemcpyDeviceToHost)) != hipSuccess)
+            return hip_fail(e, "download (wide BVH nodes, mask words)");
+        wbvh_entry_host(nodes.data(), (int64_t)nodes.size(), C, words.data(), W_ENTRY_K, W_ENTRY_FAN, W_CUT_DEPTH, sets);
+        std::memcpy(out, sets.data(), nw * 4);
+    }
+    return RT_OK;
+}
+
 void Renderer::take_counters(const unsigned long long* cnt)
 {
     last_shadow_ = (int64_t)cnt[0];
diff --git a/raytracercpp_amd/csrc/renderer.hpp b/raytracercpp_amd/csrc/renderer.hpp
--- a/raytracercpp_amd/csrc/renderer.hpp
+++ b/raytracercpp_amd/csrc/renderer.hpp
@@ -122,6 +122,7 @@
     bool risk_cap = true;
     bool scene_bound = true;
     bool tile_mask = true;
+    bool tile_start = true;
     int cut_budget = W_CUT_BUDGET;
     bool ocone = true;
     int ocone_dim = 128;
@@ -201,6 +202,7 @@
     int kernel_times(float* ms, int n);
     int band_counters(unsigned long long out[2]);
     int tile_mask(int src, uint32_t* out, int64_t cap, int32_t info[5]);
+    int tile_starts(int src, uint32_t* out, int64_t cap, int32_t info[3]);
     int debug_read(uint64_t* out, int64_t n);
     int tile_costs(uint32_t* out, int64_t n, int32_t* tiles_x, int32_t* tiles_y);
     int origin_cones(uint32_t* out, int64_t n, int32_t dims[3], float lo_ih[4]);
@@ -373,6 +375,9 @@
     int prepare_risk(KParams& P, hipStream_t stream);
     struct MaskSlot {
         DevBuf words;
+        DevBuf starts;
+        bool starts_valid = false;
+        uint32_t launches = 0;
         WMaskCam cam{};
         uint64_t cut_gen = 0;
     };
@@ -381,6 +386,7 @@
     uint64_t cut_gen_ = 0;
     MaskSlot mask_main_;
     MaskSlot* mask_last_ = nullptr;
+    bool starts_last_ = false;
     Fence cut_fence_;
     int prepare_mask(KParams& P, hipStream_t stream, MaskSlot& M);
     DevBuf d_dbg_;
diff --git a/raytracercpp_amd/csrc/wbvh.hpp b/raytracercpp_amd/csrc/wbvh.hpp
--- a/raytracercpp_amd/csrc/wbvh.hpp
+++ b/raytracercpp_amd/csrc/wbvh.hpp
@@ -617,6 +617,23 @@
     return C;
 }
 
+inline void wbvh_proj_shortcut(const float m[16], int& mode, float& w)
+{
+    mode = 0;
+    w = 1.0f;
+    bool fin = true;
+    for (int i = 0; i < 16; i++)
+        fin = fin && std::isfinite(m[i]);
+    if (fin && m[12] == 0.0f && m[13] == 0.0f && m[14] != 0.0f) {
+        volatile float mz = m[14] * -1.0f;
+        const float wt = mz + m[15];
+        if (std::isfinite(wt) && wt != 0.0f) {
+            mode = wt == 1.0f ? 1 : 2;
+            w = 1.0f / wt;
+        }
+    }
+}
+
 struct WMaskRect {
     int32_t x0, y0, x1, y1;
 };
@@ -714,6 +731,128 @@
             for (int w = R.x0 >> 5; w <= R.x1 >> 5; w++)
                 words[(size_t)y * C.wpr + w] |= wbvh_mask_word(R, w);
     }
+}
+
+constexpr int W_ENTRY_MAX = 4;
+#ifndef W_ENTRY_K
+#define W_ENTRY_K 4
+#endif
+#ifndef W_ENTRY_FAN
+#define W_ENTRY_FAN 3
+#endif
+
+struct WEntrySet {
+    uint32_t link[W_ENTRY_MAX];
+};
+
+RT_HD bool wbvh_rect_holds(const WMaskRect& R, int bx, int by)
+{
+    return bx >= R.x0 && bx <= R.x1 && by >= R.y0 && by <= R.y1;
+}
+
+RT_HD double wbvh_entry_dist(const WNode& N, const float cam[3])
+{
+    const double org[3] = {N.ox, N.oy, N.oz};
+    double s = 0.0;
+    for (int a = 0; a < 3; a++) {
+        const double st = (double)__builtin_bit_cast(float, ((N.exps >> (8 * a)) & 0xffu) << 23);
+        const double lo = org[a], hi = org[a] + 255.0 * st, c = (double)cam[a];
+        const double g = c < lo ? lo - c : (c > hi ? c - hi : 0.0);
+        s += g * g;
+    }
+    return s == s ? s : INFINITY;
+}
+
+RT_HD WEntrySet wbvh_entry_block(const WNode* nodes, int64_t nnodes, const WMaskCam& C, int bx, int by, int K, int fan,
+                                 int max_depth)
+{
+    WEntrySet S;
+    for (int i = 0; i < W_ENTRY_MAX; i++)
+        S.link[i] = W_EMPTY;
+    S.link[0] = 0u;
+    if (nnodes <= 0 || !C.valid)
+        return S;
+    K = K < 1 ? 1 : (K > W_ENTRY_MAX ? W_ENTRY_MAX : K);
+    uint32_t fn[W_ENTRY_MAX];
+    int fd[W_ENTRY_MAX];
+    bool fin[W_ENTRY_MAX];
+    int n = 1;
+    fn[0] = 0u;
+    fd[0] = 0;
+    fin[0] = false;
+    for (;;) {
+        int i = n;
+        for (int k = 0; k < n; k++)
+            if (!fin[k] && (i == n || fd[k] < fd[i]))
+                i = k;
+        if (i == n)
+            break;
+        const WNode& N = nodes[fn[i]];
+        uint32_t ch[W_WIDTH];
+        int cnt = 0;
+        bool inner = true;
+        for (int j = 0; j < W_WIDTH; j++) {
+            const uint32_t c = N.child[j];
+            if (c == W_EMPTY || !wbvh_rect_holds(wbvh_mask_rect(N, j, C), bx, by))
+                continue;
+            inner = inner && !(c & W_LEAF) && (int64_t)c < nnodes;
+            ch[cnt++] = c;
+        }
+        if (cnt == 0) {
+            for (int k = i + 1; k < n; k++) {
+                fn[k - 1] = fn[k];
+                fd[k - 1] = fd[k];
+                fin[k - 1] = fin[k];
+            }
+            n--;
+            continue;
+        }
+        if (!inner || cnt > fan || n - 1 + cnt > K || fd[i] + 1 >= max_depth) {
+            fin[i] = true;
+            continue;
+        }
+        fn[i] = ch[0];
+        fd[i]++;
+        for (int k = 1; k < cnt; k++) {
+            fn[n] = ch[k];
+            fd[n] = fd[i];
+            fin[n] = false;
+            n++;
+        }
+    }
+    if (n == 0)
+        return S;
+    double key[W_ENTRY_MAX];
+    for (int i = 0; i < n; i++)
+        key[i] = wbvh_entry_dist(nodes[fn[i]], C.cam);
+    for (int i = 1; i < n; i++)
+        for (int k = i; k > 0 && (key[k] < key[k - 1] || (key[k] == key[k - 1] && fn[k] < fn[k - 1])); k--) {
+            const double tk = key[k];
+            key[k] = key[k - 1];
+            key[k - 1] = tk;
+            const uint32_t tf = fn[k];
+            fn[k] = fn[k - 1];
+            fn[k - 1] = tf;
+        }
+    for (int i = 0; i < n; i++)
+        S.link[i] = fn[i];
+    return S;
+}
+
+inline void wbvh_entry_host(const WNode* nodes, int64_t nnodes, const WMaskCam& C, const uint32_t* words, int K, int fan,
+                            int max_depth, std::vector<uint32_t>& out)
+{
+    out.assign((size_t)C.bw * C.bh * W_ENTRY_MAX, W_EMPTY);
+    for (int by = 0; by < C.bh; by++)
+        for (int bx = 0; bx < C.bw; bx++) {
+            uint32_t* o = &out[((size_t)by * C.bw + bx) * W_ENTRY_MAX];
+            o[0] = 0u;
+            if (words && !((words[(size_t)by * C.wpr + (bx >> 5)] >> (bx & 31)) & 1u))
+                continue;
+            const WEntrySet S = wbvh_entry_block(nodes, nnodes, C, bx, by, K, fan, max_depth);
+            for (int i = 0; i < W_ENTRY_MAX; i++)
+                o[i] = S.link[i];
+        }
 }
 
 struct WRiskArgs {
@@ -956,7 +1095,7 @@
 RT_HD int wbvh_closest(const WNode* nodes, const GTri* tris, v3 o, v3 d, float m, Stack& stk, WHit& h,
                        uint32_t* work = nullptr, float hi = INFINITY, bool ties = true, float QS = 0x1p-8f,
                        const uint64_t* risk = nullptr, int rsel = 0, float rsub = 0.0f, uint32_t max_steps = 0,
-                       Feed* feed = nullptr, bool nob = false)
+                       Feed* feed = nullptr, bool nob = false, const uint32_t* start = nullptr)
 {
     static_assert(G == 1 || ((G & (G - 1)) == 0 && G <= 8 && (Stack::CAP & (Stack::CAP - 1)) == 0),
                   "a lane group: a power of two up to 8 lanes, a ring stack of 2^k entries");
@@ -994,6 +1133,12 @@
     float dropped = INFINITY;
     int sp = 0, bot = 0;
     uint32_t cur = FEED || (G > 1 && wg_lane<G>() != 0) ? W_EMPTY : 0u;
+    if (!FEED && start && cur != W_EMPTY) {
+        cur = start[0];
+        for (int i = W_ENTRY_MAX - 1; i >= 1; i--)
+            if (start[i] != W_EMPTY)
+                stk.put(slot(sp++), make_uint2(start[i], 0u));
+    }
     uint32_t nn = 0, nt = 0;
     uint32_t steps = 0;
     auto status = [&]() -> int {
diff --git a/raytracercpp_amd/renderer.py b/raytracercpp_amd/renderer.py
--- a/raytracercpp_amd/renderer.py
+++ b/raytracercpp_amd/renderer.py
@@ -411,6 +411,13 @@
         self._call("rt_tile_mask", int(src), ptr(words, _u32p), words.size, ptr(info, _i32p))
         bits = (words.reshape(bh, wpr)[:, :, None] >> np.arange(32, dtype=np.uint32)) & 1
         return bits.reshape(bh, wpr * 32)[:, :bw].astype(bool), {"on": bool(info[3]), "cut": int(info[4])}
+
+    def tile_starts(self, src=0):
+        info = np.zeros(3, np.int32)
+        self._call("rt_tile_starts", int(src), None, 0, ptr(info, _i32p))
+        sets = np.zeros((int(info[1]), int(info[0]), 4), np.uint32)
+        self._call("rt_tile_starts", int(src), ptr(sets, _u32p), sets.size, ptr(info, _i32p))
+        return sets, bool(info[2])
 
     def load_scene(self, sc: SceneData, st: RenderSettings):
         self.set_render_settings(st)
```
